# saidwivedi/TokenHMR

Hardware: AMD Instinct MI355X
Metric: crops_per_sec (higher is better)
Workload: dtype f32 (fp32 in / accumulate / out; the ViT GEMMs multiply each fp32 operand as three bf16 pieces on the bf16 MFMA pipe, six products per pair: `vit_gemm` split3; the fp32-MFMA mode is `exact_f32_mode`); 1 GPU; TokenHMR full path (ViT-H/16 + 6-layer token decoder + VQ lookup/decode + SMPL LBS), 256x256 crops, random-init weights; batch_per_gpu=64, global_batch=64, vit_depth=32, parallelism=dp1, allgather_outputs=False, vit_gemm=split3, ranks=1

## Files before the change

include/tokenhmr_hip.h:

```cpp
#ifndef TOKENHMR_HIP_H
#define TOKENHMR_HIP_H

#include <stddef.h>
#include <stdint.h>

#ifdef __cplusplus
extern "C" {
#endif

#define THMR_ABI_VERSION 5

typedef enum {
    THMR_OK = 0,
    THMR_ERR_INVALID = -1,
    THMR_ERR_HIP = -2,
    THMR_ERR_STATE = -3,
    THMR_ERR_NOMEM = -4,
    THMR_ERR_UNSUPPORTED = -5
} thmr_status;

typedef struct thmr_engine thmr_engine;

typedef struct {
    int32_t abi_version;
// ... 34 lines not shown
} thmr_smpl_desc;

typedef struct {
    float*   pred_cam;
    float*   rotmat;
    float*   betas;
    float*   cls_logits_softmax;
    float*   pred_cam_t;
    float*   focal_length;
    float*   pred_keypoints_3d;
    float*   pred_vertices;
    float*   pred_keypoints_2d;
    int32_t* token_idx;
    float*   vit_features;
    float*   token_out;
    float*   cls_logits;
    float*   pose6d;
} thmr_outputs;

enum {
    THMR_PROF_GEMM_QKV = 0, THMR_PROF_GEMM_PROJ = 1, THMR_PROF_GEMM_FC1 = 2, THMR_PROF_GEMM_FC2 = 3,
    THMR_PROF_ATTN = 4, THMR_PROF_LN = 5, THMR_PROF_PATCH = 6, THMR_PROF_DEC_KV = 7,
    THMR_PROF_HEAD = 8, THMR_PROF_LBS = 9, THMR_PROF_NUM = 10
};
typedef struct {
    double  ms;
    double  flops;
    double  bytes;
    int64_t launches;
} thmr_prof_entry;

int         thmr_abi_version(void);
const char* thmr_build_info(void);

int thmr_arena_bytes(const thmr_config* cfg, size_t* weight_bytes, size_t* scratch_bytes);

int thmr_mode_bytes(const thmr_config* cfg, int32_t vit_gemm_mode, size_t* split_weight_bytes, size_t* split_act_bytes, size_t* workspace_bytes);

int thmr_spec(const thmr_config* cfg, int32_t index, const char** name, int64_t* numel);

int thmr_create(const thmr_config* cfg, void* weight_arena_dev, void* scratch_arena_dev, thmr_engine** out);
void thmr_destroy(thmr_engine* e);
const char* thmr_last_error(const thmr_engine* e);

int thmr_load_weights(thmr_engine* e, const thmr_tensor_desc* tensors, size_t n, void* stream);
int thmr_load_smpl(thmr_engine* e, const thmr_smpl_desc* smpl, void* stream);
int thmr_finalize_weights(thmr_engine* e, int32_t assume_all_loaded, void* stream);
int thmr_weight_arena(thmr_engine* e, void** ptr_dev, size_t* bytes);

int thmr_forward(thmr_engine* e, const float* img_dev, int32_t B, const thmr_outputs* out, void* stream);

int thmr_engine_status(thmr_engine* e, void* stream);

int thmr_debug_decoder_timeline(thmr_engine* e, uint64_t* stamps_host, int32_t max_stamps, void* stream);

typedef enum {
    THMR_GEMM_F32_TILE = 0,
    THMR_GEMM_F32_TILE_SPLITK,
    THMR_GEMM_F32_RING,
    THMR_GEMM_F32_RING16,
    THMR_GEMM_S3_TILE,
    THMR_GEMM_S3_TILE_SPLITK,
    THMR_GEMM_S3_STREAM_WIDE,
    THMR_GEMM_S3_STREAM_NARROW,
    THMR_GEMM_S3_SPLITK_STREAM,
    THMR_GEMM_S3_RING
} thmr_gemm_kind;
enum { THMR_VIT_PATH_F32 = 0, THMR_VIT_PATH_SPLIT3 = 1, THMR_VIT_PATH_SPLIT3_SMALL = 2  };
enum { THMR_ATTN_F32 = 0, THMR_ATTN_F32_KEYSPLIT = 1, THMR_ATTN_F32_SPLIT3_OUT = 2, THMR_ATTN_B16 = 3 };
typedef struct thmr_gemm_choice {
    int32_t kind;
    int32_t ksplit;
} thmr_gemm_choice;
typedef struct thmr_vit_plan_desc {
    int32_t path;
    thmr_gemm_choice patch, qkv, proj, fc1, fc2, to_kv;
    int32_t attn;
    int32_t bs_blk;
    int32_t part2_in_scratch;
    int32_t tile_opts;
} thmr_vit_plan_desc;
int thmr_debug_vit_plan(const thmr_config* cfg, int32_t vit_gemm_mode, int32_t B, int32_t streams_available, thmr_vit_plan_desc* out);

int thmr_vit_forward(thmr_engine* e, const float* img_dev, int32_t B, float* feats_dev , void* stream);
int thmr_head_forward(thmr_engine* e, const float* ctx_dev , int32_t B, const thmr_outputs* out, void* stream);
int thmr_lbs_forward(thmr_engine* e, const float* rotmat_dev , const float* betas_dev ,
                     const float* cam_dev , int32_t B, float* verts_dev, float* joints_dev,
                     float* cam_t_dev, float* kp2d_dev, void* stream);
int thmr_vq_argmin(thmr_engine* e, const float* x_dev, int32_t rows, int32_t* idx_dev, float* dist_dev, void* stream);

int thmr_encode_tokens(thmr_engine* e, const float* pose_dev, int32_t B, int32_t* idx_dev, float* latent_dev, void* stream);
int thmr_vq_decode(thmr_engine* e, const float* probs_dev, int32_t B, float* pose6d_dev, void* stream);
int thmr_vq_decode_idx(thmr_engine* e, const int32_t* idx_dev, int32_t B, float* pose6d_dev, void* stream);
typedef struct thmr_tokenizer_out {
    int32_t* idx;
    float* latent;
    float* pose6d;
    float* rotmat;
    float* aa;
    float* commit_loss;
    float* perplexity;
    int32_t* code_count;
    int32_t accumulate_counts;
    int32_t reserved;
} thmr_tokenizer_out;
int thmr_tokenizer_roundtrip(thmr_engine* e, const float* pose6d_dev , int32_t B, const thmr_tokenizer_out* out, void* stream);

int thmr_op_gemm(const float* A_dev, int64_t lda, const float* W_dev, const float* bias_dev, const float* resid_dev,
                 float* C_dev, int64_t ldc, int32_t M, int32_t N, int32_t K, int32_t epi, float qscale, int32_t qcols,
                 int32_t variant, void* stream);
int thmr_op_split3(const float* src_dev, int64_t ld_src, void* dst_dev, int64_t ld_dst, int64_t rows, int32_t K, void* stream);
int thmr_op_gemm_split3(const void* A_split_dev, int64_t lda, const void* W_split_dev, int64_t ldw, const float* bias_dev,
                        const float* resid_dev, float* C_dev, int64_t ldc, int32_t M, int32_t N, int32_t K, int32_t epi,
                        float qscale, int32_t qcols, int32_t variant, void* stream);
int thmr_op_gemm_split3_out_split3(const void* A_split_dev, int64_t lda, const void* W_split_dev, int64_t ldw, const float* bias_dev,
                                   void* C_split_dev, int64_t ldcs, int32_t M, int32_t N, int32_t K, int32_t epi, float qscale,
                                   int32_t qcols, int32_t variant, void* stream);
int thmr_op_layernorm(const float* x_dev, const float* gamma_dev, const float* beta_dev, float* y_dev,
                      int32_t rows, int32_t D, float eps, int32_t relu, void* stream);
int thmr_op_vit_attention(const float* qkv_dev, float* out_dev , int32_t B, void* stream);
int thmr_op_vit_attention_variant(const float* qkv_dev, float* out_dev, int32_t B, int32_t variant, void* stream);
int thmr_op_vit_attention_split3(const float* qkv_dev, void* out_split_dev, int32_t B, void* stream);
int thmr_op_vit_attention_b16(const float* qkv_dev, void* out_dev, int32_t B, int32_t out_split, int32_t qt, void* stream);
int thmr_op_rot6d(const float* x_dev, float* R_dev, int32_t n, void* stream);
int thmr_op_aa_to_rotmat(const float* aa_dev, float* R_dev, int32_t n, void* stream);

int thmr_op_splitk_resid_ln(const float* part_dev, int32_t S, int32_t rows, int32_t D, const float* bias_dev, const float* resid_dev,
                            float* xout_dev, const float* gamma_dev, const float* beta_dev, void* y_dev, float eps, int32_t y_is_split3,
                            void* stream);
int thmr_op_add_ln64(const float* x_dev, const float* y_dev, const float* gamma_dev, const float* beta_dev, float* s_out_dev,
                     float* z_out_dev, int32_t rows, float eps, void* stream);
int thmr_op_transpose(const float* in_dev, float* out_dev, int32_t Bn, int32_t R, int32_t C, void* stream);
int thmr_op_softmax_argmax(const float* logits_dev, float* probs_or_null, int32_t* idx_or_null, int32_t rows, void* stream);
int thmr_op_cross_attn(const float* q_dev, const float* kv_dev, int64_t ldkv, int32_t koff, float* out_dev, int32_t B, void* stream);
int thmr_op_im2col_patch(const float* img_dev, void* A_dev, int32_t B, int32_t out_split, void* stream);
int thmr_op_conv3_gather(const float* in_dev, float* out_dev, const int32_t* src_or_null, int32_t Bn, int32_t Tin, int32_t Tout,
                         int32_t C, int32_t dil, int32_t prerelu, void* stream);
int thmr_op_conv_gather(const float* in_dev, float* out_dev, const int32_t* src_or_null, int32_t Bn, int32_t Tin, int32_t Tsrc,
                        int32_t Tout, int32_t C, int32_t Cp, int32_t ks, int32_t stride, int32_t pad, void* stream);
int thmr_op_conv_repack(const float* w_dev, float* wp_dev, int32_t co, int32_t ci, int32_t cp, int32_t kk, void* stream);
int thmr_op_vq_argmin_rows(const float* x_dev, const float* dot_dev, const float* cnorm_dev, int32_t* idx_dev, float* dist_or_null,
                           int32_t rows, void* stream);
int thmr_op_code_norm(const float* cb_dev, float* cn_dev, int32_t ncode, void* stream);
int thmr_op_vq_stats(const float* x_dev, const float* codebook_dev, const int32_t* idx_dev, int32_t rows, int32_t* code_count_dev,
                     int32_t accumulate, float* partial_scratch_dev, float* commit_or_null, float* perplexity_or_null, void* stream);
int thmr_op_rotmat_to_aa(const float* R_dev, float* aa_dev, int32_t n, void* stream);
int thmr_op_head_finish(int32_t kind, const float* ro_dev, int32_t ldro, const float* bpose_or_null, const float* init_pose_dev,
                        const float* init_betas_dev, const float* init_cam_dev, float* pose6d_or_null, float* rotmat_dev,
                        float* betas_dev, float* cam_dev, float* cam_t_or_null, float* focal_or_null, float focal_length, float img_size,
                        int32_t B, void* stream);
int thmr_op_decoder_init(const float* bias_dev, const float* pos_dev, float* x_dev, int32_t B, int32_t E, void* stream);

typedef struct thmr_smpl thmr_smpl;
int  thmr_smpl_create(const thmr_smpl_desc* desc, int32_t max_batch, int32_t device, thmr_smpl** out);
void thmr_smpl_destroy(thmr_smpl* m);
int  thmr_smpl_forward(thmr_smpl* m, const float* pose_dev, int32_t pose2rot, const float* betas_dev, int32_t B,
                       float* verts_dev , float* joints_dev , void* stream);

typedef struct thmr_smplh_desc {
    const float* v_template;
    const float* shapedirs;
    const float* posedirs;
    const float* J_regressor;
    const float* lbs_weights;
    const int32_t* parents;
    const int32_t* extra_verts;
    int32_t on_device;
    int32_t reserved;
} thmr_smplh_desc;
typedef struct thmr_smplh thmr_smplh;
int  thmr_smplh_create(const thmr_smplh_desc* desc, int32_t max_batch, int32_t device, thmr_smplh** out);
void thmr_smplh_destroy(thmr_smplh* m);
int  thmr_smplh_forward(thmr_smplh* m, const float* pose_dev, int32_t pose2rot, const float* betas_dev, const float* transl_dev,
                        int32_t body_only, int32_t B, float* verts_dev , float* joints_dev ,
                        void* stream);
#define THMR_MEAN_ROW_DIST_WS 256
int thmr_op_mean_row_dist(const float* a_dev, const float* b_dev, int32_t n_rows_per_item, int32_t row_lo, int32_t row_hi, int32_t B,
                          float* out_dev, float* workspace_dev, void* stream);

#define THMR_VAL_LOSS_PLAIN 0
#define THMR_VAL_LOSS_LOOSE 1
#define THMR_VAL_LOSS_WS_PER_ITEM 5
typedef struct thmr_val_loss_desc {
    double w_keypoints_2d, w_keypoints_3d, w_global_orient, w_body_pose, w_betas;
    double loose_weight;
    int32_t pelvis_id;
    int32_t mode;
    int32_t gt_pose_is_rotmat;
    int32_t reserved;
} thmr_val_loss_desc;
typedef struct thmr_val_loss_in {
    const float* pred_keypoints_2d;
    const float* pred_keypoints_3d;
    const float* pred_rotmat;
    const float* pred_betas;
    const float* gt_keypoints_2d;
    const float* gt_keypoints_3d;
    const float* gt_pose;
    const float* gt_betas;
    const float* has_global_orient;
    const float* has_body_pose;
    const float* has_betas;
    const float* valid_3d;
    const float* kp2d_thresh;
    const float* angle_thresh;
} thmr_val_loss_in;
typedef struct thmr_val_loss_out {
    float* losses;
    float* per_item;
    float* kp2d_err;
    float* angle_err;
    float* valid2d;
    float* weak2d;
    float* valid_rot;
    float* weak_rot;
    float* conf2d_used;
    float* conf3d_used;
// ... 142 lines not shown
```

tokenhmr_amd/_cabi.py:

```python
import ctypes as C
import os
import re

_HERE = os.path.dirname(os.path.abspath(__file__))
LIB_PATH = os.path.join(_HERE, "lib", "libtokenhmr_hip.so")
LIB_PATH_EXP = os.path.join(_HERE, "lib", "libtokenhmr_hip_exp.so")
HEADER = os.path.join(os.path.dirname(_HERE), "include", "tokenhmr_hip.h")

ABI_VERSION = 5
CFG_VIT_GEMM_F32, CFG_NO_PERSISTENT, CFG_HEAD_HMR2 = 1, 2, 8
PROF_NAMES = ["gemm_qkv", "gemm_proj", "gemm_fc1", "gemm_fc2", "attention", "layernorm", "patch_embed",
              "dec_kv", "head", "lbs"]


class Config(C.Structure):
    _fields_ = [("abi_version", C.c_int32), ("vit_depth", C.c_int32), ("dec_depth", C.c_int32),
                ("max_batch", C.c_int32), ("device", C.c_int32), ("flags", C.c_int32), ("reserved", C.c_int32 * 2)]


class TensorDesc(C.Structure):
    _fields_ = [("name", C.c_char_p), ("data", C.c_void_p), ("numel", C.c_int64),
                ("on_device", C.c_int32), ("reserved", C.c_int32)]


# ... 56 lines not shown


class JpegPlan(C.Structure):
    _fields_ = [(n, C.c_int32) for n in ("height", "width", "components", "h_samp", "v_samp", "win_x0", "win_y0", "win_w", "win_h", "mcu_row0",
                                         "mcu_rows_kept", "mcu_rows_decoded")] + \
               [(n, C.c_int32 * 3) for n in ("bx0", "by0", "bw", "bh", "coef_block")] + [("n_blocks", C.c_int32), ("quant", (C.c_uint16 * 64) * 3)]


class JpegItem(C.Structure):
    _fields_ = [("coef", C.c_void_p), ("plan", C.POINTER(JpegPlan)), ("win_x0", C.c_int32), ("win_y0", C.c_int32), ("win_w", C.c_int32),
                ("win_h", C.c_int32), ("out_dev", C.c_void_p), ("row_stride", C.c_int64)]


ERR_INVALID, ERR_HIP, ERR_STATE, ERR_NOMEM, ERR_UNSUPPORTED = -1, -2, -3, -4, -5

RENDER_MAX_LIGHTS = 16
RENDER_PER_IMAGE, RENDER_ONE_IMAGE = 0, 1
LIGHT_DIRECTIONAL, LIGHT_POINT = 0, 1


class RenderLight(C.Structure):
    _fields_ = [("type", C.c_int32), ("vec", C.c_float * 3), ("color", C.c_float * 3), ("intensity", C.c_float)]


class RenderDesc(C.Structure):
    _fields_ = [("width", C.c_int32), ("height", C.c_int32), ("fx", C.c_float), ("fy", C.c_float), ("cx", C.c_float), ("cy", C.c_float),
                ("znear", C.c_float), ("samples", C.c_int32), ("mode", C.c_int32), ("translate_first", C.c_int32),
                ("rot", C.c_float * 9), ("base_color", C.c_float * 3), ("mesh_colors", C.POINTER(C.c_float)), ("bg_color", C.c_float * 3),
                ("metallic", C.c_float), ("roughness", C.c_float), ("ambient", C.c_float * 3), ("n_lights", C.c_int32),
                ("lights", RenderLight * RENDER_MAX_LIGHTS), ("out_channels", C.c_int32), ("img_mean", C.c_float * 3),
                ("img_std", C.c_float * 3), ("ids_dev", C.c_void_p)]


SHEET_IMAGE, SHEET_FRONT, SHEET_SIDE = 1, 2, 4
SHEET_KEYPOINTS, SHEET_RECORDS, SHEET_RECORD_WORDS = 44, 49, 12


class SheetDesc(C.Structure):
    _fields_ = [("n", C.c_int32), ("width", C.c_int32), ("height", C.c_int32), ("img_res", C.c_int32), ("panels", C.c_int32),
                ("nrow", C.c_int32), ("padding", C.c_int32), ("canvas_width", C.c_int32), ("canvas_height", C.c_int32)]


class GemmChoice(C.Structure):
    _fields_ = [("kind", C.c_int32), ("ksplit", C.c_int32)]


GEMM_KINDS = ["f32_tile", "f32_tile_splitk", "f32_ring", "f32_ring16", "s3_tile", "s3_tile_splitk", "s3_stream_wide", "s3_stream_narrow",
              "s3_splitk_stream", "s3_ring"]
VIT_PATHS = ["f32", "split3", "split3_small"]
ATTN_KINDS = ["f32", "f32_keysplit", "f32_split3_out", "b16"]


class VitPlanDesc(C.Structure):
    _fields_ = [("path", C.c_int32)] + [(n, GemmChoice) for n in ("patch", "qkv", "proj", "fc1", "fc2", "to_kv")] + \
               [("attn", C.c_int32), ("bs_blk", C.c_int32), ("part2_in_scratch", C.c_int32), ("tile_opts", C.c_int32)]


class TokenizerOut(C.Structure):
    _fields_ = [("idx", C.c_void_p), ("latent", C.c_void_p), ("pose6d", C.c_void_p), ("rotmat", C.c_void_p), ("aa", C.c_void_p),
                ("commit_loss", C.c_void_p), ("perplexity", C.c_void_p), ("code_count", C.c_void_p), ("accumulate_counts", C.c_int32),
                ("reserved", C.c_int32)]


class ProfEntry(C.Structure):
    _fields_ = [("ms", C.c_double), ("flops", C.c_double), ("bytes", C.c_double), ("launches", C.c_int64)]


def declared_functions():
    with open(HEADER) as f:
        text = f.read()
    text = re.sub(r"/\*.*?\*/", "", text, flags=re.S)
    return {name: ret.strip() for ret, name in re.findall(r"([A-Za-z_][\w \t*]*?)\b(thmr_[a-z0-9_]+)\s*\(", text)}


def declared_symbols():
    return sorted(declared_functions())


_libs = {}

ROWOPS_SYMBOLS = ("thmr_op_splitk_resid_ln", "thmr_op_add_ln64", "thmr_op_transpose", "thmr_op_softmax_argmax", "thmr_op_cross_attn",
                  "thmr_op_im2col_patch", "thmr_op_conv3_gather", "thmr_op_conv_gather", "thmr_op_conv_repack", "thmr_op_vq_argmin_rows",
                  "thmr_op_code_norm", "thmr_op_head_finish", "thmr_op_decoder_init")

TOKENIZER_RT_SYMBOLS = ("thmr_vq_decode_idx", "thmr_tokenizer_roundtrip", "thmr_op_vq_stats", "thmr_op_rotmat_to_aa")

SMPLH_SYMBOLS = ("thmr_smplh_create", "thmr_smplh_destroy", "thmr_smplh_forward", "thmr_op_mean_row_dist")

LOSS_SYMBOLS = ("thmr_val_loss", "thmr_op_token_ce")

FRAMES_SYMBOLS = ("thmr_cropper_run_frames",)

JPEG_SYMBOLS = ("thmr_jpeg_probe", "thmr_jpeg_entropy_decode", "thmr_jpeg_decode_host", "thmr_jpeg_create", "thmr_jpeg_destroy",
                "thmr_jpeg_last_error", "thmr_jpeg_decode_batch")


def load(exp=None):
    if exp is None:
        exp = os.environ.get("THMR_LIB", "") == "exp"
    if isinstance(exp, str):
        path = os.path.abspath(exp)
        exp = path
    else:
        exp = bool(exp)
        path = LIB_PATH_EXP if exp else LIB_PATH
    if exp in _libs:
        return _libs[exp]
    if not os.path.exists(path):
        raise RuntimeError(
            f"{path} not found: the HIP extension is not built. Run `python __graft_entry__.py` "
            "(hipcc --offload-arch=gfx950). There is no CPU fallback for the product path.")
    try:
        import torch
    except ImportError:
        pass
    lib = C.CDLL(path)
    declared = declared_functions()
    restypes = {"int": C.c_int, "void": None, "const char*": C.c_char_p}
    for name, ret in declared.items():
        if ret not in restypes:
            raise RuntimeError(f"tokenhmr_hip.h declares {name} as returning '{ret}': _cabi.load() knows {sorted(restypes)}")
        if hasattr(lib, name):
            getattr(lib, name).restype = restypes[ret]
    older = isinstance(exp, str) and lib.thmr_abi_version() in (3, 4)
    missing = [s for s in sorted(declared) if not hasattr(lib, s) and not (older and s in ("thmr_mode_bytes",))
               and not (isinstance(exp, str) and s in ("thmr_renderer_sheet", "thmr_debug_vit_plan") + ROWOPS_SYMBOLS + TOKENIZER_RT_SYMBOLS + FRAMES_SYMBOLS + JPEG_SYMBOLS)]
    if missing:
        raise RuntimeError(f"libtokenhmr_hip.so lacks symbols declared in tokenhmr_hip.h: {missing}")
    vp, i32, i64, f32, sz = C.c_void_p, C.c_int32, C.c_int64, C.c_float, C.c_size_t
    lib.thmr_last_error.argtypes = [vp]
    lib.thmr_arena_bytes.argtypes = [C.POINTER(Config), C.POINTER(sz), C.POINTER(sz)]
    lib.thmr_spec.argtypes = [C.POINTER(Config), i32, C.POINTER(C.c_char_p), C.POINTER(i64)]
    if hasattr(lib, "thmr_mode_bytes"):
        lib.thmr_mode_bytes.argtypes = [C.POINTER(Config), i32, C.POINTER(sz), C.POINTER(sz), C.POINTER(sz)]
    lib.thmr_create.argtypes = [C.POINTER(Config), vp, vp, C.POINTER(vp)]
    lib.thmr_destroy.argtypes = [vp]
    lib.thmr_load_weights.argtypes = [vp, C.POINTER(TensorDesc), sz, vp]
    lib.thmr_load_smpl.argtypes = [vp, C.POINTER(SmplDesc), vp]
    lib.thmr_finalize_weights.argtypes = [vp, i32, vp]
    lib.thmr_weight_arena.argtypes = [vp, C.POINTER(vp), C.POINTER(sz)]
    lib.thmr_forward.argtypes = [vp, vp, i32, C.POINTER(Outputs), vp]
    lib.thmr_engine_status.argtypes = [vp, vp]
    lib.thmr_debug_decoder_timeline.argtypes = [vp, C.POINTER(C.c_uint64), i32, vp]
    if hasattr(lib, "thmr_debug_vit_plan"):
        lib.thmr_debug_vit_plan.argtypes = [C.POINTER(Config), i32, i32, i32, C.POINTER(VitPlanDesc)]
    lib.thmr_vit_forward.argtypes = [vp, vp, i32, vp, vp]
    lib.thmr_head_forward.argtypes = [vp, vp, i32, C.POINTER(Outputs), vp]
    lib.thmr_lbs_forward.argtypes = [vp, vp, vp, vp, i32, vp, vp, vp, vp, vp]
    lib.thmr_vq_argmin.argtypes = [vp, vp, i32, vp, vp, vp]
    lib.thmr_encode_tokens.argtypes = [vp, vp, i32, vp, vp, vp]
    lib.thmr_vq_decode.argtypes = [vp, vp, i32, vp, vp]
    lib.thmr_op_gemm.argtypes = [vp, i64, vp, vp, vp, vp, i64, i32, i32, i32, i32, f32, i32, i32, vp]
    lib.thmr_op_layernorm.argtypes = [vp, vp, vp, vp, i32, i32, f32, i32, vp]
    lib.thmr_op_vit_attention.argtypes = [vp, vp, i32, vp]
    lib.thmr_op_vit_attention_variant.argtypes = [vp, vp, i32, i32, vp]
    lib.thmr_op_vit_attention_split3.argtypes = [vp, vp, i32, vp]
    lib.thmr_op_vit_attention_b16.argtypes = [vp, vp, i32, i32, i32, vp]
    lib.thmr_op_split3.argtypes = [vp, i64, vp, i64, i64, i32, vp]
    lib.thmr_op_gemm_split3.argtypes = [vp, i64, vp, i64, vp, vp, vp, i64, i32, i32, i32, i32, f32, i32, i32, vp]
    lib.thmr_op_gemm_split3_out_split3.argtypes = [vp, i64, vp, i64, vp, vp, i64, i32, i32, i32, i32, f32, i32, i32, vp]
    lib.thmr_op_rot6d.argtypes = [vp, vp, i32, vp]
    lib.thmr_op_aa_to_rotmat.argtypes = [vp, vp, i32, vp]
    if hasattr(lib, "thmr_op_splitk_resid_ln"):
        lib.thmr_op_splitk_resid_ln.argtypes = [vp, i32, i32, i32, vp, vp, vp, vp, vp, vp, f32, i32, vp]
        lib.thmr_op_add_ln64.argtypes = [vp, vp, vp, vp, vp, vp, i32, f32, vp]
        lib.thmr_op_transpose.argtypes = [vp, vp, i32, i32, i32, vp]
        lib.thmr_op_softmax_argmax.argtypes = [vp, vp, vp, i32, vp]
        lib.thmr_op_cross_attn.argtypes = [vp, vp, i64, i32, vp, i32, vp]
        lib.thmr_op_im2col_patch.argtypes = [vp, vp, i32, i32, vp]
        lib.thmr_op_conv3_gather.argtypes = [vp, vp, vp, i32, i32, i32, i32, i32, i32, vp]
        lib.thmr_op_conv_gather.argtypes = [vp, vp, vp, i32, i32, i32, i32, i32, i32, i32, i32, i32, vp]
        lib.thmr_op_conv_repack.argtypes = [vp, vp, i32, i32, i32, i32, vp]
        lib.thmr_op_vq_argmin_rows.argtypes = [vp, vp, vp, vp, vp, i32, vp]
        lib.thmr_op_code_norm.argtypes = [vp, vp, i32, vp]
        lib.thmr_op_head_finish.argtypes = [i32, vp, i32, vp, vp, vp, vp, vp, vp, vp, vp, vp, vp, f32, f32, i32, vp]
        lib.thmr_op_decoder_init.argtypes = [vp, vp, vp, i32, i32, vp]
    if hasattr(lib, "thmr_tokenizer_roundtrip"):
        lib.thmr_vq_decode_idx.argtypes = [vp, vp, i32, vp, vp]
        lib.thmr_tokenizer_roundtrip.argtypes = [vp, vp, i32, C.POINTER(TokenizerOut), vp]
        lib.thmr_op_vq_stats.argtypes = [vp, vp, vp, i32, vp, i32, vp, vp, vp, vp]
        lib.thmr_op_rotmat_to_aa.argtypes = [vp, vp, i32, vp]
    if hasattr(lib, "thmr_smplh_create"):
        lib.thmr_smplh_create.argtypes = [C.POINTER(SmplhDesc), i32, i32, C.POINTER(vp)]
        lib.thmr_smplh_destroy.argtypes = [vp]
        lib.thmr_smplh_forward.argtypes = [vp, vp, i32, vp, vp, i32, i32, vp, vp, vp]
        lib.thmr_op_mean_row_dist.argtypes = [vp, vp, i32, i32, i32, i32, vp, vp, vp]
    if hasattr(lib, "thmr_val_loss"):
        lib.thmr_val_loss.argtypes = [C.POINTER(ValLossDesc), C.POINTER(ValLossIn), i32, C.POINTER(ValLossOut), vp, vp]
        lib.thmr_op_token_ce.argtypes = [vp, vp, i32, vp, vp, vp]
    lib.thmr_smpl_create.argtypes = [C.POINTER(SmplDesc), i32, i32, C.POINTER(vp)]
    lib.thmr_smpl_destroy.argtypes = [vp]
    lib.thmr_smpl_forward.argtypes = [vp, vp, i32, vp, i32, vp, vp, vp]
    lib.thmr_eval_pose.argtypes = [vp, vp, i32, i32, vp, i32, i32, i32, vp, vp, i32, i32, vp, vp, vp, vp, vp]
    lib.thmr_regress_joints.argtypes = [vp, vp, i32, i32, i32, vp, vp]
    lib.thmr_cropper_create.argtypes = [i32, C.POINTER(vp)]
    lib.thmr_cropper_destroy.argtypes = [vp]
    lib.thmr_cropper_last_error.argtypes = [vp]
    lib.thmr_cropper_run.argtypes = [vp, vp, i32, i32, i64, C.POINTER(CropDesc), i32, i32, i32, C.POINTER(f32), C.POINTER(f32), vp, vp]
    if hasattr(lib, "thmr_cropper_run_frames"):
        lib.thmr_cropper_run_frames.argtypes = [vp, C.POINTER(FrameCrop), i32, i32, i32, C.POINTER(f32), C.POINTER(f32), vp, vp]
    if hasattr(lib, "thmr_jpeg_probe"):
        lib.thmr_jpeg_probe.argtypes = [vp, sz, C.POINTER(JpegInfo)]
        lib.thmr_jpeg_entropy_decode.argtypes = [vp, sz, C.POINTER(i32), vp, i64, C.POINTER(JpegPlan)]
        lib.thmr_jpeg_decode_host.argtypes = [vp, sz, C.POINTER(i32), i32, vp, i64]
        lib.thmr_jpeg_create.argtypes = [i32, C.POINTER(vp)]
        lib.thmr_jpeg_destroy.argtypes = [vp]
        lib.thmr_jpeg_last_error.argtypes = [vp]
        lib.thmr_jpeg_decode_batch.argtypes = [vp, C.POINTER(JpegItem), i32, i32, vp]
    lib.thmr_renderer_create.argtypes = [i32, vp, i32, i32, C.POINTER(vp)]
    lib.thmr_renderer_destroy.argtypes = [vp]
    lib.thmr_renderer_last_error.argtypes = [vp]
    lib.thmr_renderer_run.argtypes = [vp, C.POINTER(RenderDesc), vp, vp, i32, vp, vp, vp]
    if hasattr(lib, "thmr_renderer_sheet"):
        lib.thmr_renderer_sheet.argtypes = [vp, C.POINTER(SheetDesc), vp, vp, vp, vp, vp, vp, vp, vp]
    lib.thmr_pack_records.argtypes = [C.POINTER(Outputs), i32, vp, vp]
    lib.thmr_bcast_weights.argtypes = [vp, vp, i32, vp]
    lib.thmr_allgather_records.argtypes = [vp, vp, i32, vp, vp]
    lib.thmr_prof_enable.argtypes = [vp, i32]
    lib.thmr_set_vit_gemm.argtypes = [vp, i32, vp]
    lib.thmr_get_vit_gemm.argtypes = [vp]
    lib.thmr_prof_collect.argtypes = [vp, C.POINTER(ProfEntry), i32]
    if lib.thmr_abi_version() != ABI_VERSION and not older:
        raise RuntimeError("libtokenhmr_hip.so ABI version mismatch")
    _libs[exp] = lib
    return lib


class EngineError(RuntimeError):
    pass


def check(rc, engine=None, lib=None):
    if rc != 0:
        lib = lib if lib is not None else load()
        msg = lib.thmr_last_error(engine)
        raise EngineError(f"tokenhmr_hip error {rc}: {msg.decode() if msg else '?'}")


def raise_error(rc, what, msg, error=EngineError, by_code=None):
    raise (by_code or {}).get(rc, error)(f"{what} error {rc}: {msg.decode() if msg else '?'}")


class Handle:
    error, error_by_code, no_gpu_error = EngineError, None, RuntimeError

    @classmethod
    def cuda_device(cls, device, needs_gpu, resolve):
        import torch
        dev = torch.device(device)
        if dev.type != "cuda":
            raise cls.no_gpu_error(needs_gpu)
        return torch.device("cuda", torch.cuda.current_device()) if resolve and dev.index is None else dev

    def __init__(self, device, stem, needs_gpu, last_error=None):
        self.device = self.cuda_device(device, needs_gpu, resolve=False)
        self._needs_gpu = needs_gpu
        self.lib = load()
        self._stem, self._per_handle = stem, last_error is None
        self._last_error = getattr(self.lib, last_error or stem + "_last_error")
# ... 26 lines not shown
```

tokenhmr_amd/csrc/common.h:

```cpp
#pragma once
#include <hip/hip_runtime.h>
#include <stdint.h>

typedef float f32x4 __attribute__((ext_vector_type(4)));
typedef float f32x16 __attribute__((ext_vector_type(16)));

#include <cstdlib>
#ifdef THMR_EXPERIMENTS
inline const char* thmr_knob(const char* name) { return getenv(name); }
#else
inline const char* thmr_knob(const char*) { return nullptr; }
#endif

#define THMR_WAVE 64

enum GemmEpi {
    EPI_NONE = 0,
    EPI_BIAS = 1,
    EPI_BIAS_GELU = 2,
    EPI_BIAS_RELU = 3,
    EPI_BIAS_RESID = 4,
    EPI_BIAS_QSCALE = 5,
    EPI_BIAS_POS = 6,
    EPI_NUM = 7
// ... 149 lines not shown
    const uint32_t u2 = __float_as_uint(r2);
    L = (u2 + 0x7fffu + ((u2 >> 16) & 1u)) & 0xffff0000u;
    if (nan) H = M = L = 0x7fc00000u;
}
__device__ __forceinline__ void split3_of(float x, uint32_t& h, uint32_t& m, uint32_t& l) {
    uint32_t H, M, L;
    split3_hi(x, H, M, L);
    h = H >> 16; m = M >> 16; l = L >> 16;
}
__device__ __forceinline__ uint32_t cvt_pk_bf16(float lo, float hi) {
    typedef __bf16 bf16x2_t __attribute__((ext_vector_type(2)));
    typedef float f32x2_t __attribute__((ext_vector_type(2)));
    return __builtin_bit_cast(uint32_t, __builtin_convertvector(f32x2_t{lo, hi}, bf16x2_t));
}
__device__ __forceinline__ void split3_pair(float x0, float x1, uint32_t& H, uint32_t& M, uint32_t& L) {
#pragma clang fp contract(off)
    typedef float f32x2_t __attribute__((ext_vector_type(2)));
    H = cvt_pk_bf16(x0, x1);
    f32x2_t r = f32x2_t{x0, x1} - f32x2_t{__uint_as_float(H << 16), __uint_as_float(H & 0xffff0000u)};
    M = cvt_pk_bf16(r.x, r.y);
    r = r - f32x2_t{__uint_as_float(M << 16), __uint_as_float(M & 0xffff0000u)};
    L = cvt_pk_bf16(r.x, r.y);
}
__device__ __forceinline__ void store_split3_quad(char* row, int c, f32x4 v) {
    typedef uint32_t u32x2 __attribute__((ext_vector_type(2)));
    uint32_t H[2], M[2], L[2];
    split3_pair(v[0], v[1], H[0], M[0], L[0]);
    split3_pair(v[2], v[3], H[1], M[1], L[1]);
    char* o = row + (c >> 3) * 48 + (c & 4) * 2;
    *reinterpret_cast<u32x2*>(o) = u32x2{H[0], H[1]};
    *reinterpret_cast<u32x2*>(o + 16) = u32x2{M[0], M[1]};
    *reinterpret_cast<u32x2*>(o + 32) = u32x2{L[0], L[1]};
}

__device__ __forceinline__ void store_split3_oct(char* row, int c, f32x4 lo, f32x4 hi) {
    typedef uint32_t u32x4_t __attribute__((ext_vector_type(4)));
    uint32_t H[4], M[4], L[4];
    split3_pair(lo[0], lo[1], H[0], M[0], L[0]);
    split3_pair(lo[2], lo[3], H[1], M[1], L[1]);
    split3_pair(hi[0], hi[1], H[2], M[2], L[2]);
    split3_pair(hi[2], hi[3], H[3], M[3], L[3]);
    u32x4_t* o = reinterpret_cast<u32x4_t*>(row + (c >> 3) * 48);
    o[0] = u32x4_t{H[0], H[1], H[2], H[3]};
    o[1] = u32x4_t{M[0], M[1], M[2], M[3]};
    o[2] = u32x4_t{L[0], L[1], L[2], L[3]};
}

__device__ __forceinline__ float wave_sum(float v) {
#pragma unroll
    for (int o = 32; o > 0; o >>= 1) v += __shfl_xor(v, o, 64);
    return v;
}
__device__ __forceinline__ float wave_max(float v) {
#pragma unroll
    for (int o = 32; o > 0; o >>= 1) v = fmaxf(v, __shfl_xor(v, o, 64));
    return v;
}

__device__ __forceinline__ void st_dev(float* p, float v) { __hip_atomic_store(p, v, __ATOMIC_RELAXED, __HIP_MEMORY_SCOPE_AGENT); }
__device__ __forceinline__ float ld_dev(const float* p) { return __hip_atomic_load(p, __ATOMIC_RELAXED, __HIP_MEMORY_SCOPE_AGENT); }
__device__ __forceinline__ f32x4 ld_dev4(const float* p) {
    typedef float f32x2_t __attribute__((ext_vector_type(2)));
    union { unsigned long long u; f32x2_t f; } a, b;
    a.u = __hip_atomic_load(reinterpret_cast<const unsigned long long*>(p), __ATOMIC_RELAXED, __HIP_MEMORY_SCOPE_AGENT);
    b.u = __hip_atomic_load(reinterpret_cast<const unsigned long long*>(p) + 1, __ATOMIC_RELAXED, __HIP_MEMORY_SCOPE_AGENT);
    return f32x4{a.f.x, a.f.y, b.f.x, b.f.y};
}

struct MixerLayerW {
    const float *ln1w, *ln1b, *wt1, *bt1, *wt2, *bt2, *ln2w, *ln2b, *wc1, *bc1, *wc2, *bc2;
};
struct MixerParams {
    MixerLayerW L[4];
    const float *tln_w, *tln_b;
    const float *wn, *bn, *nln_w, *nln_b;
    const float* mt;
    float* out;
};


struct DecLayerW {
    const float *n0w, *n0b, *wv, *wo1, *bo1;
    const float *n1w, *n1b, *wq, *wo2, *bo2;
    const float *n2w, *n2b, *w1, *b1, *w2, *b2;
};
struct DecParams {
    DecLayerW L[6];
    const float *tok_bias, *pos;
    const float* kv;
    const float *ro_w, *ro_b, *mt_w, *mt_b;
    float *dx, *dv, *dq, *dca, *dff, *ro, *mt;
    unsigned* sync;
    unsigned* host_err;
    int64_t ldkv;
    int depth, B;
    int timeline;
    int debug_fail;
    int barrier_a2a;
    int max_blocks;
    MixerParams mx;
    float* mixy[2];
    int mixer_cluster;
};

constexpr int THMR_HEAD_TOKEN = 0, THMR_HEAD_HMR2 = 1;
constexpr int THMR_HMR2_RO_ROWS = 157, THMR_HMR2_RO_LD = 160;
int launch_decoder_fused(const DecParams& p, hipStream_t s, int head = THMR_HEAD_TOKEN);
int decoder_max_coresident_blocks(int device, int head = THMR_HEAD_TOKEN);
int launch_hmr2_finish(const float* ro, int ldro, const float* init_pose, const float* init_betas, const float* init_cam, float* pose6d,
                       float* rotmat, float* betas, float* cam, float* cam_t, float* focal, float focal_length, float img_size, int B,
                       hipStream_t s);

int launch_mixer_fused(const MixerParams& p, int B, hipStream_t s);

int launch_gemm(const GemmArgs& a, int epi, int variant, hipStream_t s);
int launch_gemm_splitk(const GemmArgs& a, int variant, int ksplit, float* part, hipStream_t s);
int launch_gemm_ring(const GemmArgs& a, int epi, int ring, int ksplit, float* part, hipStream_t s);
int launch_gemm_ring16(const GemmArgs& a, int epi, hipStream_t s);
int launch_split3(const float* src, int64_t ld_src, void* dst, int64_t ld_dst, int64_t rows, int K, hipStream_t s);
int launch_gemm_split3(const GemmArgs& a, int epi, int variant, hipStream_t s);
int launch_gemm_split3_splitk(const GemmArgs& a, int ksplit, float* part, hipStream_t s);
size_t gemm_split3_persist_ws_bytes();
bool gemm_split3_persist_ok(const GemmArgs& a);
int launch_gemm_split3_persist(const GemmArgs& a, int epi, int mode, void* ws, hipStream_t s);
bool gemm_split3_persist_narrow_ok(const GemmArgs& a);
int launch_gemm_split3_persist_narrow(const GemmArgs& a, int epi, void* ws, hipStream_t s);
int launch_gemm_split3_splitk_stream(const GemmArgs& a, int ksplit, float* part, void* ws, hipStream_t s);
int gemm_split3_persist_error(void* ws, hipStream_t s, unsigned* err_out);
int gemm_split3_persist_bind_host_err(void* ws, unsigned* const* host_err_slot, hipStream_t s);
void* gemm_split3_persist_op_ws(hipStream_t s);
int launch_split16_tiles(const GemmArgs& a, int epi, int shape, hipStream_t s);
int launch_split16_persist(const GemmArgs& a, int epi, void* ws, bool narrow, hipStream_t s);
int launch_split16_tiles_tail(const GemmArgs& a, int epi, int cus, bool tail8, hipStream_t s);
int launch_gemm_split3_ring(const GemmArgs& a, int epi, int ksplit, float* part, hipStream_t s);
int launch_layernorm_split3(const float* x, const float* g, const float* b, void* y_split, int rows, int D, float eps, hipStream_t s);
int launch_gemm_skinny(const GemmArgs& a, int epi, hipStream_t s);
int launch_vit_attention(const float* qkv, float* out, int B, hipStream_t s);
int launch_vit_attention_split3(const float* qkv, void* out_split, int B, hipStream_t s);
int launch_vit_attention_keysplit(const float* qkv, float* out, int B, hipStream_t s);
int launch_vit_attention_variant(const float* qkv, float* out, int B, int variant, hipStream_t s);
int launch_vit_attention_b16(const float* qkv, void* out, int B, bool out_split, int qt, hipStream_t s);
int launch_layernorm(const float* x, const float* g, const float* b, float* y, int rows, int D, float eps, int relu,
                     hipStream_t s);
int launch_splitk_epilogue(const GemmArgs& a, int epi, const float* part, int S, hipStream_t s);
int launch_splitk_resid_ln(const float* part, int S, int rows, int D, const float* bias, const float* resid, float* xout,
                           const float* gamma, const float* beta, float* y, float eps, hipStream_t s, bool y_is_split3 = false);
int launch_add_ln64(const float* x, const float* y, const float* g, const float* b, float* s_out, float* z_out, int rows,
                    float eps, hipStream_t s);
int launch_im2col_patch(const float* img, float* A, int B, hipStream_t s);
int launch_im2col_patch_split3(const float* img, void* A_split, int B, hipStream_t s);
int launch_transpose(const float* in, float* out, int Bn, int R, int C, hipStream_t s);
int launch_softmax_argmax2048(const float* logits, float* probs, int32_t* idx, int rows, hipStream_t s);
int launch_conv3_gather(const float* in, float* out, const int32_t* src, int Bn, int Tin, int Tout, int C, int dil,
                        int prerelu, hipStream_t s);
int launch_conv_repack(const float* w, float* wp, int co, int ci, int kk, hipStream_t s);
int launch_conv_gather_general(const float* in, float* out, const int32_t* src, int Bn, int Tin, int Tsrc, int Tout, int C,
                               int Cp, int ks, int stride, int pad, hipStream_t s);
int launch_conv_repack_pad(const float* w, float* wp, int co, int ci, int cp, int kk, hipStream_t s);
int launch_decoder_init(const float* bias, const float* pos, float* x, int B, int E, hipStream_t s);
int launch_cross_attn(const float* q, const float* kv, int64_t ldkv, int koff, float* out, int B, hipStream_t s);
int launch_assemble(const float* ro, int ldro, const float* bpose, const float* init_pose, const float* init_betas,
                    const float* init_cam, float* pose6d, float* rotmat, float* betas, float* cam, float* cam_t,
                    float* focal, float focal_length, float img_size, int B, hipStream_t s);
int launch_rot6d(const float* x, float* R, int n, hipStream_t s);
int launch_aa_to_rotmat(const float* aa, float* R, int n, hipStream_t s);
int launch_cam_t(const float* cam, float* cam_t, float focal_length, float img_size, int B, hipStream_t s);
int launch_vq_argmin_rows(const float* x, const float* dot, const float* cnorm, int32_t* idx, float* dist, int rows,
                          hipStream_t s);
int launch_code_norm(const float* cb, float* cn, int ncode, hipStream_t s);
int launch_vq_lookup(const int32_t* idx, const float* x, const float* cb, float* out, int B, unsigned* bad_flag, hipStream_t s);
int vq_stats_partials(int rows);
int launch_vq_stats(const float* x, const float* cb, const int32_t* idx, int rows, int32_t* count, int accumulate, float* partial,
                    float* commit, float* perplexity, unsigned* bad_flag, hipStream_t s);
int launch_rotmat_to_aa(const float* R, float* aa, int n, hipStream_t s);
int launch_eval_pose(const float* pred, const float* gt, int nj, int gt_stride, const int32_t* kp, int nkp, int pelvis_ind,
                     int pelvis_mode, float* mpjpe, float* re, float* pelv, int B, hipStream_t s);
int launch_eval_pve(const float* pv, const float* gv, const float* pelv, int nv, float* pve, int B, hipStream_t s);
int launch_regress_joints(const float* J, const float* verts, int nj, int nv, float* out, int B, hipStream_t s);
constexpr int kMeanRowDistWs = 256;
int launch_mean_row_dist(const float* a, const float* b, int n, int row_lo, int row_hi, int B, float* out, float* partial, hipStream_t s);
struct ValLossArgs {
    const float *pred_kp2d, *pred_kp3d, *pred_rotmat, *pred_betas;
    const float *gt_kp2d, *gt_kp3d, *gt_pose, *gt_betas;
    const float *has_global_orient, *has_body_pose, *has_betas;
    const float *valid_3d, *kp2d_thresh, *angle_thresh;
    float *losses, *per_item, *kp2d_err, *angle_err;
    float *valid2d, *weak2d, *valid_rot, *weak_rot;
    float *conf2d_used, *conf3d_used, *has_betas_used;
    double* running;
    float* partial;
    double w[5];
// ... 36 lines not shown
```

tokenhmr_amd/csrc/decoder_fused.hip:

```cpp
#include <cstdlib>

#include "mixer_device.h"

namespace {

constexpr int E = 1024, INNER = 512, DMLP = 1024, TOKK = 192, NHEAD = 8;
constexpr int NBLK = 64, NWAVE = 8, NS = 8;
constexpr float LN_EPS = 1e-5f;

struct GridSync {
    unsigned* w;
    unsigned base;
    unsigned n;
    unsigned* host_err;
    int a2a;
};

template <class PF>
__device__ __forceinline__ bool grid_barrier(GridSync& gs, int tid, volatile int* s_ok, PF&& pf) {
    asm volatile("s_waitcnt vmcnt(0) lgkmcnt(0)" ::: "memory");
    pf();
    __syncthreads();
    gs.n += 1;
    const unsigned epoch = gs.base + gs.n;
// ... 164 lines not shown
                if (m < B) {
                    float o = v[r];
                    if constexpr (EPI != 0) o = o + bv;
                    if constexpr (EPI == 2) o = gelu_erf(o);
                    if constexpr (EPI == 4) o = ld_dev(resid + (int64_t)m * ldc + n) + o;
                    st_dev(C + (int64_t)m * ldc + n, o);
                }
            }
        }
        __syncthreads();
    }
}

__device__ __forceinline__ void gemv_multi(const float* __restrict__ A, const float* __restrict__ W0, const float* __restrict__ b0, float* C0,
                                           const float* __restrict__ W1, const float* __restrict__ b1, float* C1, int n_ro, int n_all, int B,
                                           float (*red)[64][4], int tid, bool dev_c1) {
    const int lane = tid & 63, wave = __builtin_amdgcn_readfirstlane(tid >> 6), l15 = lane & 15, g = lane >> 4;
    const int kbeg = wave * (E / NWAVE);
    const int nsub = (B + 15) >> 4, G = gridDim.x;
    auto wptr = [&](int vt) -> const float* {
        return vt < n_ro ? W0 + (int64_t)min(vt * 16 + l15, 31) * E + kbeg + g * 4
                         : W1 + (int64_t)((vt - n_ro) * 16 + l15) * E + kbeg + g * 4;
    };
    const int lanes_of_b = min(nsub, G);
    for (int mt = blockIdx.x % lanes_of_b; mt < nsub; mt += lanes_of_b) {
        const int first = blockIdx.x / lanes_of_b, step = G / lanes_of_b;
        if (first >= step) continue;
        const int m0 = mt * 16;
        const float* ap = A + (int64_t)min(m0 + l15, B - 1) * E + kbeg + g * 4;
        f32x4 xq[NS], wq[NS], wn[NS];
#pragma unroll
        for (int s = 0; s < NS; ++s) xq[s] = ld_dev4(ap + s * 16);
        int vt = first;
        if (vt < n_all) {
            const float* wp = wptr(vt);
#pragma unroll
            for (int s = 0; s < NS; ++s) wq[s] = *reinterpret_cast<const f32x4*>(wp + s * 16);
        }
#pragma unroll 1
        for (; vt < n_all; vt += step) {
            const int nxt = vt + step;
            if (nxt < n_all) {
                const float* wp = wptr(nxt);
#pragma unroll
                for (int s = 0; s < NS; ++s) wn[s] = *reinterpret_cast<const f32x4*>(wp + s * 16);
            }
            f32x4 acc = {0.f, 0.f, 0.f, 0.f};
#pragma unroll
            for (int s = 0; s < NS; ++s)
#pragma unroll
                for (int t = 0; t < 4; ++t) acc = __builtin_amdgcn_mfma_f32_16x16x4f32(xq[s][t], wq[s][t], acc, 0, 0, 0);
            *reinterpret_cast<f32x4*>(&red[wave][lane][0]) = acc;
            __syncthreads();
            if (wave == 0) {
                f32x4 v = *reinterpret_cast<const f32x4*>(&red[0][lane][0]);
#pragma unroll
                for (int w = 1; w < NWAVE; ++w) v += *reinterpret_cast<const f32x4*>(&red[w][lane][0]);
                const bool ro = vt < n_ro;
                const int n = (ro ? vt : vt - n_ro) * 16 + l15, N = ro ? 31 : 10240, ldc = ro ? 32 : 10240;
                if (n < N) {
                    const float bv = (ro ? b0 : b1)[n];
                    float* C = ro ? C0 : C1;
#pragma unroll
                    for (int r = 0; r < 4; ++r) {
                        const int m = m0 + g * 4 + r;
                        if (m < B) {
                            if (!ro && dev_c1) st_dev(&C[(int64_t)m * ldc + n], v[r] + bv);
                            else C[(int64_t)m * ldc + n] = v[r] + bv;
                        }
                    }
                }
            }
            __syncthreads();
#pragma unroll
            for (int s = 0; s < NS; ++s) wq[s] = wn[s];
        }
    }
}

}

namespace {

__device__ __forceinline__ void cross_attn_stage(const DecParams& p, int layer, int tid, float* pl ) {
    const int lane = tid & 63, l15 = lane & 15, g = lane >> 4;
    const int gwave = __builtin_amdgcn_readfirstlane(tid >> 6) * gridDim.x + blockIdx.x;
    for (int item = gwave; item < p.B * NHEAD; item += gridDim.x * NWAVE) {
        const int b = item >> 3, h = item & 7;
        const f32x4 qv = ld_dev4(p.dq + (int64_t)b * INNER + h * 64 + l15 * 4);
        const float* kb = p.kv + (int64_t)b * TOKK * p.ldkv + layer * 2 * INNER + h * 64 + l15 * 4;
        float s3[3] = {0.f, 0.f, 0.f};
        const int64_t cstride = (int64_t)48 * p.ldkv;
        const float* kp = kb + (int64_t)g * p.ldkv;
        auto load8 = [&](const float* src, f32x4 (&dst)[12]) {
#pragma unroll
            for (int i = 0; i < 12; ++i) dst[i] = *reinterpret_cast<const f32x4*>(src + (int64_t)(i * 4) * p.ldkv);
        };
        auto score8 = [&](const f32x4 (&kk)[12], int c) {
#pragma unroll
            for (int i = 0; i < 12; ++i) {
                float d = kk[i][0] * qv[0];
                d = fmaf(kk[i][1], qv[1], d);
                d = fmaf(kk[i][2], qv[2], d);
                d = fmaf(kk[i][3], qv[3], d);
                d += __shfl_xor(d, 1, 64);
                d += __shfl_xor(d, 2, 64);
                d += __shfl_xor(d, 4, 64);
                d += __shfl_xor(d, 8, 64);
                const int idx = c * 12 + i;
                const bool mine = l15 == (idx & 15);
                const float sv = d * 0.125f;
                if (mine && (idx >> 4) == 0) s3[0] = sv;
                if (mine && (idx >> 4) == 1) s3[1] = sv;
                if (mine && (idx >> 4) == 2) s3[2] = sv;
            }
        };
        {
            f32x4 ka[12], kc[12];
            load8(kp, ka);
#pragma unroll 1
            for (int c = 0; c < 4; c += 2) {
                load8(kp + (int64_t)(c + 1) * cstride, kc);
                score8(ka, c);
                if (c + 2 < 4) load8(kp + (int64_t)(c + 2) * cstride, ka);
                score8(kc, c + 1);
            }
        }
        const float m = wave_max(fmaxf(fmaxf(s3[0], s3[1]), s3[2]));
        float e3[3];
#pragma unroll
        for (int j = 0; j < 3; ++j) {
            e3[j] = expf(s3[j] - m);
            pl[g * 48 + j * 16 + l15] = e3[j];
        }
        const float sum = wave_sum((e3[0] + e3[1]) + e3[2]);
        const float* vp = kb + INNER + (int64_t)g * p.ldkv;
        const float* wl = pl + g * 48;
        f32x4 acc = {0.f, 0.f, 0.f, 0.f};
        auto pv8 = [&](const f32x4 (&vv)[12], int c) {
#pragma unroll
            for (int i = 0; i < 12; ++i) {
                const float w = wl[c * 12 + i];
#pragma unroll
                for (int e = 0; e < 4; ++e) acc[e] = fmaf(w, vv[i][e], acc[e]);
            }
        };
        {
            f32x4 va[12], vc[12];
            load8(vp, va);
#pragma unroll 1
            for (int c = 0; c < 4; c += 2) {
                load8(vp + (int64_t)(c + 1) * cstride, vc);
                pv8(va, c);
                if (c + 2 < 4) load8(vp + (int64_t)(c + 2) * cstride, va);
                pv8(vc, c + 1);
            }
        }
#pragma unroll
        for (int e = 0; e < 4; ++e) {
            acc[e] += __shfl_xor(acc[e], 16, 64);
            acc[e] += __shfl_xor(acc[e], 32, 64);
        }
        if (g == 0) {
            const float inv = 1.0f / sum;
            float* o = p.dca + (int64_t)b * INNER + h * 64 + l15 * 4;
#pragma unroll
            for (int e = 0; e < 4; ++e) st_dev(o + e, acc[e] * inv);
        }
    }
}

__device__ __forceinline__ bool mixer_cluster_stage(const DecParams& p, GridSync& gs, int tid, volatile int* s_ok, float* Y, float* U, float* Xl,
                                                    float* redbuf) {
    using namespace mixer;
    const int lane = tid & 63, wave = __builtin_amdgcn_readfirstlane(tid >> 6), l15 = lane & 15, g = lane >> 4;
    const int wg = blockIdx.x;
    const int per_crop = p.mixer_cluster, tpw = 10 / per_crop;
    const bool active = wg < per_crop * p.B;
    const int b = wg / per_crop, t0 = (wg - b * per_crop) * tpw * 16, nrow = tpw * 16;
    if (active) {
        f32x4 o[5];
        trans_ln<true>(p.mt + (int64_t)b * (T * H), p.mx.tln_w, p.mx.tln_b, redbuf, tid, lane, wave, o);
#pragma unroll
        for (int i = 0; i < 5; ++i) {
            const int e0 = (i * NT + tid) * 4, t = e0 >> 6, h = e0 & 63;
            if (t >= t0 && t < t0 + nrow) *reinterpret_cast<f32x4*>(&Xl[(t - t0) * LD + h]) = o[i];
        }
    }
    __syncthreads();
#pragma unroll 1
    for (int l = 0; l < 4; ++l) {
        const MixerLayerW& w = p.mx.L[l];
        float* yg = p.mixy[l & 1] + (int64_t)b * (T * H);
        if (active) {
            const float gamma = w.ln1w[lane], beta = w.ln1b[lane];
            for (int r = wave; r < nrow; r += NW) st_dev(yg + (t0 + r) * H + lane, ln_row_value(Xl[r * LD + lane], gamma, beta));
        }
        if (!grid_barrier(gs, tid, s_ok)) return false;
        if (active) {
            for (int idx = tid; idx < T * H / 4; idx += NT) {
                const int t = idx >> 4, h = (idx & 15) * 4;
                *reinterpret_cast<f32x4*>(&Y[t * LD + h]) = ld_dev4(yg + idx * 4);
            }
            __syncthreads();
#pragma unroll 1
            for (int tile = wave; tile < 16; tile += NW) token_mix1_tile(Y, U, w, tile, l15, g);
            __syncthreads();
#pragma unroll 1
            for (int tile = wave; tile < 4 * tpw; tile += NW) {
                const int tt = tile >> 2;
                token_mix2_tile(U, Xl + tt * 16 * LD, Y + (t0 + tt * 16) * LD, w, (tile & 3) * 16, t0 + tt * 16, l15, g);
            }
            __syncthreads();
#pragma unroll 1
            for (int tt = 0; tt < tpw; ++tt)
                channel_mix_tile_8waves(Y + (t0 + tt * 16) * LD, Xl + tt * 16 * LD, U, w, wave, lane, l15, g);
        }
    }
    if (active)
        for (int tt = wave; tt < tpw; tt += NW) norm_layer_tile(Xl + tt * 16 * LD, p.mx.out + ((int64_t)b * T + t0 + tt * 16) * H, p.mx, l15, g);
    return true;
}

template <int HEAD>
__global__ __launch_bounds__(NWAVE * 64) void decoder_persistent_kernel(DecParams p) {
    constexpr bool TOKEN = HEAD == THMR_HEAD_TOKEN;
    __shared__ __attribute__((aligned(16))) float mixY[TOKEN ? mixer::T * mixer::LD : 4];
    __shared__ __attribute__((aligned(16))) float mixU[TOKEN ? mixer::H * mixer::LD : 4];
    __shared__ __attribute__((aligned(16))) float mixX[TOKEN ? 80 * mixer::LD : 4];
    __shared__ float mixred[mixer::NW];
    static_assert(mixer::NW == NWAVE, "the distributed mixer tail uses the decoder kernel's 8 waves");
    __shared__ __attribute__((aligned(16))) float red[NWAVE][64][4];
    __shared__ RowStat rowstat;
    __shared__ unsigned s_base;
    __shared__ int s_ok;
    const int tid = threadIdx.x;
    if (tid == 0) s_base = __hip_atomic_load(&p.sync[1], __ATOMIC_RELAXED, __HIP_MEMORY_SCOPE_AGENT);
    __syncthreads();
    GridSync gs{p.sync, s_base, 0, p.host_err, p.barrier_a2a};
    bool ok = true;
#ifdef THMR_EXPERIMENTS
    if (p.debug_fail && blockIdx.x == 0 && tid == 0) {
        __hip_atomic_store(&gs.w[3], 1u, __ATOMIC_RELAXED, __HIP_MEMORY_SCOPE_AGENT);
        if (gs.host_err) __hip_atomic_store(gs.host_err, 1u, __ATOMIC_RELAXED, __HIP_MEMORY_SCOPE_SYSTEM);
    }
#endif
    const int B = p.B;
    unsigned long long* stamp = (p.timeline && blockIdx.x == 0 && tid == 0) ? reinterpret_cast<unsigned long long*>(p.sync + 16) : nullptr;
    int nstamp = 0;
#define THMR_STAMP() do { if (stamp) stamp[nstamp++] = wall_clock64(); } while (0)
    THMR_STAMP();

    for (int i = blockIdx.x * (NWAVE * 64) + tid; i < B * E; i += gridDim.x * NWAVE * 64) {
        const int c = i & (E - 1);
        st_dev(p.dx + i, p.tok_bias[c] + p.pos[c]);
    }
    THMR_STAMP();
    WPre pre;
    pre.item = -1;
    ok = grid_barrier(gs, tid, &s_ok, [&] { prefetch_w(pre, p.L[0].wv, E, INNER, B, tid); });
    THMR_STAMP();
    for (int l = 0; ok && l < p.depth; ++l) {
        const DecLayerW& w = p.L[l];
        gemv_stage<true, 0>(p.dx, E, w.n0w, w.n0b, w.wv, E, nullptr, nullptr, p.dv, INNER, INNER, B, red, &rowstat, tid, pre);
        THMR_STAMP();
        if (!(ok = grid_barrier(gs, tid, &s_ok, [&] { prefetch_w(pre, w.wo1, INNER, E, B, tid); }))) break;
        THMR_STAMP();
        gemv_stage<false, 4>(p.dv, INNER, nullptr, nullptr, w.wo1, INNER, w.bo1, p.dx, p.dx, E, E, B, red, &rowstat, tid, pre);
        THMR_STAMP();
        if (!(ok = grid_barrier(gs, tid, &s_ok, [&] { prefetch_w(pre, w.wq, E, INNER, B, tid); }))) break;
        THMR_STAMP();
        gemv_stage<true, 0>(p.dx, E, w.n1w, w.n1b, w.wq, E, nullptr, nullptr, p.dq, INNER, INNER, B, red, &rowstat, tid, pre);
        THMR_STAMP();
        pre.item = -1;
        if (!(ok = grid_barrier(gs, tid, &s_ok))) break;
        THMR_STAMP();
        cross_attn_stage(p, l, tid, &red[__builtin_amdgcn_readfirstlane(tid >> 6)][0][0]);
        THMR_STAMP();
        if (!(ok = grid_barrier(gs, tid, &s_ok, [&] { prefetch_w(pre, w.wo2, INNER, E, B, tid); }))) break;
        THMR_STAMP();
        gemv_stage<false, 4>(p.dca, INNER, nullptr, nullptr, w.wo2, INNER, w.bo2, p.dx, p.dx, E, E, B, red, &rowstat, tid, pre);
        THMR_STAMP();
        if (!(ok = grid_barrier(gs, tid, &s_ok, [&] { prefetch_w(pre, w.w1, E, DMLP, B, tid); }))) break;
        THMR_STAMP();
        gemv_stage<true, 2>(p.dx, E, w.n2w, w.n2b, w.w1, E, w.b1, nullptr, p.dff, DMLP, DMLP, B, red, &rowstat, tid, pre);
        THMR_STAMP();
        if (!(ok = grid_barrier(gs, tid, &s_ok, [&] { prefetch_w(pre, w.w2, DMLP, E, B, tid); }))) break;
        THMR_STAMP();
        gemv_stage<false, 4>(p.dff, DMLP, nullptr, nullptr, w.w2, DMLP, w.b2, p.dx, p.dx, E, E, B, red, &rowstat, tid, pre);
        THMR_STAMP();
        if (l + 1 < p.depth) {
            if (!(ok = grid_barrier(gs, tid, &s_ok, [&] { prefetch_w(pre, p.L[l + 1].wv, E, INNER, B, tid); }))) break;
        } else {
            pre.item = -1;
            if (!(ok = grid_barrier(gs, tid, &s_ok))) break;
        }
        THMR_STAMP();
    }
    if constexpr (!TOKEN) {
        if (ok) gemv_stage<false, 1>(p.dx, E, nullptr, nullptr, p.ro_w, E, p.ro_b, nullptr, p.ro, THMR_HMR2_RO_LD, THMR_HMR2_RO_LD, B, red, &rowstat, tid, pre);
        THMR_STAMP();
    } else {
        if (ok) {
            gemv_multi(p.dx, p.ro_w, p.ro_b, p.ro, p.mt_w, p.mt_b, p.mt, 2, 2 + 640, B, red, tid, p.mixer_cluster != 0);
        }
        THMR_STAMP();
        if (ok && p.mixer_cluster != 0) {
            ok = grid_barrier(gs, tid, &s_ok);
            if (ok) ok = mixer_cluster_stage(p, gs, tid, &s_ok, mixY, mixU, mixX, mixred);
        }
        THMR_STAMP();
    }
    __syncthreads();
    if (tid == 0) {
        const unsigned old = __hip_atomic_fetch_add(&p.sync[2], 1u, __ATOMIC_ACQ_REL, __HIP_MEMORY_SCOPE_AGENT);
        if (old == gridDim.x - 1) {
            __hip_atomic_store(&p.sync[1], gs.base + gs.n, __ATOMIC_RELAXED, __HIP_MEMORY_SCOPE_AGENT);
            __hip_atomic_store(&p.sync[2], 0u, __ATOMIC_RELEASE, __HIP_MEMORY_SCOPE_AGENT);
        }
    }
}

}

constexpr int kDecMinGrid = 128;
int launch_decoder_fused(const DecParams& p, hipStream_t s, int head) {
    if (p.B < 1 || p.depth < 1 || p.depth > 6) return -1;
    if (head == THMR_HEAD_HMR2) {
        if (p.mixer_cluster != 0) return -1;
        const int nsub = (p.B + 15) / 16;
        int grid = NBLK * (nsub < 4 ? nsub : 4);
        if (p.max_blocks > 0 && grid > p.max_blocks) grid = p.max_blocks;
        if (grid > 256) grid = 256;
        hipLaunchKernelGGL(decoder_persistent_kernel<THMR_HEAD_HMR2>, dim3(grid), dim3(NWAVE * 64), 0, s, p);
        return hipGetLastError() == hipSuccess ? 0 : -2;
    }
    if (head != THMR_HEAD_TOKEN) return -1;
    const int nsub = (p.B + 15) / 16;
    int grid = NBLK * (nsub < 4 ? nsub : 4);
    static const int min_grid = [] { const char* e = thmr_knob("THMR_DEC_MIN_GRID"); return e ? atoi(e) : kDecMinGrid; }();
    if (grid < min_grid) grid = min_grid;
    if (p.mixer_cluster != 0 && p.mixer_cluster != 10 && p.mixer_cluster != 5 && p.mixer_cluster != 2) return -1;
    if (grid < p.mixer_cluster * p.B) grid = p.mixer_cluster * p.B;
    if (p.max_blocks > 0 && grid > p.max_blocks) grid = p.max_blocks;
    if (grid > 256) grid = 256;
    if (grid < p.mixer_cluster * p.B) return -1;
#ifdef THMR_EXPERIMENTS
    static const bool coop = [] { const char* e = thmr_knob("THMR_DEC_COOP"); return e && e[0] == '1'; }();
    if (coop) {
        DecParams pc = p;
        void* args[] = {&pc};
        return hipLaunchCooperativeKernel(reinterpret_cast<const void*>(&decoder_persistent_kernel<THMR_HEAD_TOKEN>), dim3(grid), dim3(NWAVE * 64), args, 0, s) == hipSuccess ? 0 : -2;
    }
#endif
    hipLaunchKernelGGL(decoder_persistent_kernel<THMR_HEAD_TOKEN>, dim3(grid), dim3(NWAVE * 64), 0, s, p);
    return hipGetLastError() == hipSuccess ? 0 : -2;
}

int decoder_max_coresident_blocks(int device, int head) {
    int cus = 0, per_cu = 0;
    if (hipDeviceGetAttribute(&cus, hipDeviceAttributeMultiprocessorCount, device) != hipSuccess || cus < 1) return -2;
    const hipError_t q = head == THMR_HEAD_HMR2
        ? hipOccupancyMaxActiveBlocksPerMultiprocessor(&per_cu, decoder_persistent_kernel<THMR_HEAD_HMR2>, NWAVE * 64, 0)
        : hipOccupancyMaxActiveBlocksPerMultiprocessor(&per_cu, decoder_persistent_kernel<THMR_HEAD_TOKEN>, NWAVE * 64, 0);
    if (q != hipSuccess || per_cu < 1) return -2;
    return cus;
}
```

tokenhmr_amd/csrc/engine.hip:

```cpp
#include <hip/hip_runtime.h>

#include <cmath>
#include <cstdio>
#include <cstdlib>
#include <cstring>
#include <map>
#include <mutex>
#include <string>
#include <unordered_map>
#include <vector>

#include "../../include/tokenhmr_hip.h"
#include "abi_util.h"
#include "common.h"
#include "vit_plan.h"

namespace {

constexpr int HEADS = 16;
constexpr int E = 1024, DEC_MLP = 1024;
constexpr int TN = 160, NCLS = 2048, HID = 64, HID_INTER = 256, TOK_INTER = 64, MIX = 4;
constexpr int CODE = 256, VQW = 512, VQJ = 21;
constexpr float VIT_EPS = 1e-6f, LN_EPS = 1e-5f;
constexpr int kFusedHeadMaxB = 128;
// ... 573 lines not shown
            if (plan.attn == THMR_ATTN_F32_KEYSPLIT) LAUNCH_OK(launch_vit_attention_keysplit(big, h, B, st));
            else LAUNCH_OK(launch_vit_attention(big, h, B, st));
        }
        if (int rc = resid_linear_ln(THMR_PROF_GEMM_PROJ, plan.proj, h, DIM, w.pw, w.pb, w.n2w, w.n2b, h)) return rc;
        {
            ProfScope ps(e, st, THMR_PROF_GEMM_FC1, 2.0 * M * DIM * (double)MLP, 4.0 * ((double)M * DIM + (double)DIM * MLP + (double)M * MLP), (i & 3) == 0);
            GemmArgs a = mk(h, DIM, w.f1w, DIM, w.f1b, nullptr, 0, big, MLP, M, MLP, DIM);
            LAUNCH_OK(run_gemm(e, plan.fc1, a, EPI_BIAS_GELU, nullptr, st));
        }
        if (int rc = resid_linear_ln(THMR_PROF_GEMM_FC2, plan.fc2, big, MLP, w.f2w, w.f2b, nxt_w, nxt_b, last && feats_out ? feats_out : h))
            return rc;
    }
    return 0;
}


int vq_tiny_variant(const thmr_engine* e, int B) { return (e->tiny_gemm && B * TOK <= kSmallM) ? 11 : -1; }

int vq_decode_convs(thmr_engine* e, int B, float* bpose, hipStream_t st) {
    auto& so = e->so;
    const int tv = vq_tiny_variant(e, B);
    float* G[2] = {e->S(so.gat), e->S(so.gat2)};
    float *x0 = e->S(so.act0), *x1 = e->S(so.act1), *hid = e->S(so.act2);
    const int32_t* inv = reinterpret_cast<const int32_t*>(e->warena + e->o_inv);
    auto scatter = [&](GemmArgs& a, float* dst, const int32_t* table, int tin, int tout, int dil, int relu) {
        a.cs_out = dst; a.cs_inv = table; a.cs_tin = tin; a.cs_tout = tout; a.cs_dil = dil; a.cs_relu = relu;
    };
    auto conv = [&](int id, const float* opnd, int T, const float* bias, float* plain) {
        const int ci = kConv3Ci[id], co = kConv3Co[id];
        return mk(opnd, 3 * ci, e->warena + e->convp[id], 3 * ci, bias, nullptr, 0, plain, co, B * T, co, 3 * ci);
    };
    int cur = 0;
    {
        GemmArgs a = conv(0, G[cur], 160, e->hot.conv_b[0], nullptr);
        scatter(a, G[cur ^ 1], inv + 0 * 160, 160, e->vq_len[1], 1, 0);
        LAUNCH_OK(launch_gemm(a, EPI_BIAS_RELU, tv, st));
        cur ^= 1;
    }
    for (int i = 0; i < 4; ++i) {
        const int T = e->vq_len[i + 1];
        GemmArgs a = conv(1 + i, G[cur], T, e->hot.conv_b[1 + i], i == 3 ? x0 : nullptr);
        if (i < 3) scatter(a, G[cur ^ 1], inv + (i + 1) * 160, T, e->vq_len[i + 2], 1, 0);
        else scatter(a, G[cur ^ 1], nullptr, VQJ, VQJ, 3, 1);
        LAUNCH_OK(launch_gemm(a, EPI_BIAS_RELU, tv, st));
        cur ^= 1;
    }
    const int Tq = VQJ;
    float* res = x0;
    float* nres = x1;
    for (int blk = 0; blk < 2; ++blk) {
        {
            GemmArgs a = conv(5 + blk, G[cur], Tq, e->hot.conv_b[5 + blk], hid);
            LAUNCH_OK(launch_gemm(a, EPI_BIAS_RELU, tv, st));
        }
        GemmArgs a = mk(hid, VQW, e->hot.res_w[blk], VQW, e->hot.res_b[blk], res, VQW, blk == 0 ? nres : nullptr, VQW, B * Tq, VQW, VQW);
        scatter(a, G[cur ^ 1], nullptr, Tq, Tq, 1, blk == 0 ? 1 : 0);
        LAUNCH_OK(launch_gemm(a, EPI_BIAS_RESID, tv, st));
        cur ^= 1;
        std::swap(res, nres);
    }
    {
        GemmArgs a = conv(7, G[cur], Tq, e->hot.conv_b[7], nullptr);
        scatter(a, G[cur ^ 1], nullptr, Tq, Tq, 1, 0);
        LAUNCH_OK(launch_gemm(a, EPI_BIAS, tv, st));
        cur ^= 1;
    }
    GemmArgs a = conv(8, G[cur], Tq, e->hot.conv_b[8], bpose);
    LAUNCH_OK(launch_gemm(a, EPI_BIAS, tv, st));
    return 0;
}

int vq_decode(thmr_engine* e, const float* probs, int B, float* bpose, hipStream_t st) {
    GemmArgs a = mk(probs, NCLS, e->warena + e->o_cbT, NCLS, nullptr, nullptr, 0, nullptr, CODE, B * TN, CODE, NCLS);
    a.cs_out = e->S(e->so.gat); a.cs_inv = nullptr; a.cs_tin = 160; a.cs_tout = 160; a.cs_dil = 1; a.cs_relu = 0;
    LAUNCH_OK(launch_gemm(a, EPI_NONE, vq_tiny_variant(e, B), st));
    return vq_decode_convs(e, B, bpose, st);
}

int vq_decode_idx(thmr_engine* e, const int32_t* idx, const float* x, int B, float* bpose, hipStream_t st) {
    LAUNCH_OK(launch_vq_lookup(idx, x, e->W("quantizer.codebook"), e->S(e->so.gat), B, e->host_err ? e->host_err + 2 : nullptr, st));
    return vq_decode_convs(e, B, bpose, st);
}

int head_forward(thmr_engine* e, const float* ctx, int B, const thmr_outputs* out, hipStream_t st) {
    auto& so = e->so;
    const int M = B * TOK;
    float* big = e->S(so.big);
    const int ldkv = e->dec_depth * 2 * INNER;
    {
        ProfScope ps(e, st, THMR_PROF_DEC_KV, 2.0 * M * DIM * (double)ldkv, 4.0 * ((double)M * DIM + (double)ldkv * DIM + (double)M * ldkv));
        const VitPlan plan = plan_of(e, B);
        if (plan.to_kv.kind != THMR_GEMM_F32_TILE) {
            LAUNCH_OK(launch_split3(ctx, DIM, e->split_act, DIM, M, DIM, st));
            GemmArgs a = mk(reinterpret_cast<const float*>(e->split_act), DIM, reinterpret_cast<const float*>(e->kv_s), DIM, nullptr, nullptr, 0, big, ldkv, M, ldkv, DIM);
            a.tile_opts = plan.tile_opts;
            LAUNCH_OK(run_gemm(e, plan.to_kv, a, EPI_NONE, nullptr, st));
        } else {
            GemmArgs a = mk(ctx, DIM, e->warena + e->o_kv_all, DIM, nullptr, nullptr, 0, big, ldkv, M, ldkv, DIM);
            LAUNCH_OK(run_gemm(e, plan.to_kv, a, EPI_NONE, nullptr, st));
        }
    }
    ProfScope ps_head(e, st, THMR_PROF_HEAD, e->hmr2 ? 2.0 * B * (6.0 * 4.2e6 + 0.16e6) : 2.0 * B * (6.0 * 4.2e6 + 116.7e6 + 167.8e6 + 705.0e6), 0);
    float *dx = e->S(so.dx), *dh = e->S(so.dh), *dv = e->S(so.dv), *dq = e->S(so.dq), *dca = e->S(so.dca), *dff = e->S(so.dff);
    const std::string T = "smpl_head.transformer.";
    const std::string C = "smpl_head.decpose.";
    float* ro = e->S(so.ro);
    float *mt = e->S(so.mt), *cf = e->S(so.cf), *cf2 = e->S(so.cf2);
    const bool fused_head = !e->legacy_head && B <= kFusedHeadMaxB;
    bool mixer_in_decoder = false;
    if (fused_head) {
        DecParams d = e->dec;
        d.B = B;
        if (e->hmr2) {
            d.mixer_cluster = 0;
            LAUNCH_OK(launch_decoder_fused(d, st, THMR_HEAD_HMR2));
        } else {
            const int slots = d.max_blocks < 256 ? d.max_blocks : 256;
            d.mixer_cluster = !e->mixer_cluster ? 0 : 10 * B <= slots ? 10 : 5 * B <= slots ? 5 : 2 * B <= slots ? 2 : 0;
            mixer_in_decoder = d.mixer_cluster != 0;
            d.mx = e->mix;
            d.mixy[0] = cf; d.mixy[1] = cf2;
            LAUNCH_OK(launch_decoder_fused(d, st));
        }
    } else {
    LAUNCH_OK(launch_decoder_init(e->W(T + "to_token_embedding.bias"), e->W(T + "pos_embedding"), dx, B, E, st));
    for (int l = 0; l < e->dec_depth; ++l) {
        const std::string p = T + "transformer.layers." + std::to_string(l) + ".";
        LAUNCH_OK(launch_layernorm(dx, e->W(p + "0.norm.weight"), e->W(p + "0.norm.bias"), dh, B, E, LN_EPS, 0, st));
        {
            GemmArgs a = mk(dh, E, e->W(p + "0.fn.to_qkv.weight") + (size_t)2 * INNER * E, E, nullptr, nullptr, 0, dv, INNER, B, INNER, E);
            LAUNCH_OK(launch_gemm_skinny(a, EPI_NONE, st));
        }
        {
            GemmArgs a = mk(dv, INNER, e->W(p + "0.fn.to_out.0.weight"), INNER, e->W(p + "0.fn.to_out.0.bias"), dx, E, dx, E, B, E, INNER);
            LAUNCH_OK(launch_gemm_skinny(a, EPI_BIAS_RESID, st));
        }
        LAUNCH_OK(launch_layernorm(dx, e->W(p + "1.norm.weight"), e->W(p + "1.norm.bias"), dh, B, E, LN_EPS, 0, st));
        {
            GemmArgs a = mk(dh, E, e->W(p + "1.fn.to_q.weight"), E, nullptr, nullptr, 0, dq, INNER, B, INNER, E);
            LAUNCH_OK(launch_gemm_skinny(a, EPI_NONE, st));
        }
        LAUNCH_OK(launch_cross_attn(dq, big, ldkv, l * 2 * INNER, dca, B, st));
        {
            GemmArgs a = mk(dca, INNER, e->W(p + "1.fn.to_out.0.weight"), INNER, e->W(p + "1.fn.to_out.0.bias"), dx, E, dx, E, B, E, INNER);
            LAUNCH_OK(launch_gemm_skinny(a, EPI_BIAS_RESID, st));
        }
        LAUNCH_OK(launch_layernorm(dx, e->W(p + "2.norm.weight"), e->W(p + "2.norm.bias"), dh, B, E, LN_EPS, 0, st));
        {
            GemmArgs a = mk(dh, E, e->W(p + "2.fn.net.0.weight"), E, e->W(p + "2.fn.net.0.bias"), nullptr, 0, dff, DEC_MLP, B, DEC_MLP, E);
            LAUNCH_OK(launch_gemm_skinny(a, EPI_BIAS_GELU, st));
        }
        {
            GemmArgs a = mk(dff, DEC_MLP, e->W(p + "2.fn.net.3.weight"), DEC_MLP, e->W(p + "2.fn.net.3.bias"), dx, E, dx, E, B, E, DEC_MLP);
            LAUNCH_OK(launch_gemm_skinny(a, EPI_BIAS_RESID, st));
        }
    }
    if (e->hmr2) {
        GemmArgs a = mk(dx, E, e->warena + e->o_ro_w, E, e->warena + e->o_ro_b, nullptr, 0, ro, THMR_HMR2_RO_LD, B, THMR_HMR2_RO_LD, E);
        LAUNCH_OK(launch_gemm_skinny(a, EPI_BIAS, st));
    } else {
        {
            GemmArgs a = mk(dx, E, e->warena + e->o_ro_w, E, e->warena + e->o_ro_b, nullptr, 0, ro, 32, B, 31, E);
            LAUNCH_OK(launch_gemm_skinny(a, EPI_BIAS, st));
        }
        {
            GemmArgs a = mk(dx, E, e->W(C + "mixer_trans.ff.0.weight"), E, e->W(C + "mixer_trans.ff.0.bias"), nullptr, 0, mt, TN * HID, B, TN * HID, E);
            LAUNCH_OK(launch_gemm_skinny(a, EPI_BIAS, st));
        }
    }
    }
    if (out && out->token_out) HIP_OK(hipMemcpyAsync(out->token_out, dx, sizeof(float) * B * E, hipMemcpyDeviceToDevice, st));
    if (e->hmr2) {
        float* rot = (out && out->rotmat) ? out->rotmat : e->S(so.rot);
        float* betas = (out && out->betas) ? out->betas : e->S(so.betas);
        float* cam = (out && out->pred_cam) ? out->pred_cam : e->S(so.cam);
        float* camt = (out && out->pred_cam_t) ? out->pred_cam_t : e->S(so.camt);
        LAUNCH_OK(launch_hmr2_finish(ro, THMR_HMR2_RO_LD, e->hot.init_pose, e->hot.init_betas, e->hot.init_cam, out ? out->pose6d : nullptr,
                                     rot, betas, cam, camt, out ? out->focal_length : nullptr, FOCAL, IMG, B, st));
        return 0;
    }
    const int R = B * TN;
    float *nl = e->S(so.nl), *nl2 = e->S(so.nl2);
    if (fused_head) {
        if (!mixer_in_decoder) LAUNCH_OK(launch_mixer_fused(e->mix, B, st));
    } else {
        LAUNCH_OK(launch_layernorm(mt, e->W(C + "mixer_trans.ff.1.weight"), e->W(C + "mixer_trans.ff.1.bias"), cf, B, TN * HID, LN_EPS, 1, st));
        for (int m = 0; m < MIX; ++m) {
            const std::string p = C + "mixer_head." + std::to_string(m) + ".";
            float *y1 = e->S(so.y1), *tT = e->S(so.tT), *u = e->S(so.u), *yt = e->S(so.yt), *y = e->S(so.y), *s = e->S(so.s),
                  *z0 = e->S(so.z0), *zh = e->S(so.zh);
            LAUNCH_OK(launch_layernorm(cf, e->W(p + "layernorm1.weight"), e->W(p + "layernorm1.bias"), y1, R, HID, LN_EPS, 0, st));
            LAUNCH_OK(launch_transpose(y1, tT, B, TN, HID, st));
            {
                GemmArgs a = mk(tT, TN, e->W(p + "MLP_token.ff.0.weight"), TN, e->W(p + "MLP_token.ff.0.bias"), nullptr, 0, u, TOK_INTER, B * HID, TOK_INTER, TN);
                LAUNCH_OK(launch_gemm(a, EPI_BIAS_GELU, -1, st));
// ... 439 lines not shown
    char* p = e->split_w;
    for (int i = 0; i < e->vit_depth; ++i) {
        const VitBlockW& w = e->vitw[i];
        auto conv = [&](const float* src, int rows, int K, const char*& out) -> int {
            out = p;
            const int rc = launch_split3(src, K, p, K, rows, K, st);
            p += (size_t)rows * K * 6;
            return rc;
        };
        LAUNCH_OK(conv(w.qkvw, 3 * DIM, DIM, e->vitw_s[i].qkv));
        LAUNCH_OK(conv(w.pw, DIM, DIM, e->vitw_s[i].proj));
        LAUNCH_OK(conv(w.f1w, MLP, DIM, e->vitw_s[i].fc1));
        LAUNCH_OK(conv(w.f2w, DIM, MLP, e->vitw_s[i].fc2));
    }
    e->kv_s = p;
    LAUNCH_OK(launch_split3(e->warena + e->o_kv_all, DIM, p, DIM, (int64_t)kv_rows, DIM, st));
    p += kv_rows * DIM * 6;
    e->pe_s = p;
    LAUNCH_OK(launch_split3(e->hot.pe_w, 768, p, 768, DIM, 768, st));
    return 0;
}

int thmr_finalize_weights(thmr_engine* e, int32_t assume_all_loaded, void* stream) {
    if (!e) return fail(e, THMR_ERR_INVALID, "null engine");
    hipStream_t st = static_cast<hipStream_t>(stream);
    if (!assume_all_loaded) {
        for (auto& n : e->required)
            if (!e->slots[n].loaded) return fail(e, THMR_ERR_STATE, "missing tensor '" + n + "' (strict load)");
        if (!e->smpl_loaded) return fail(e, THMR_ERR_STATE, "SMPL constants not loaded (thmr_load_smpl)");
    }
    int32_t* flags = reinterpret_cast<int32_t*>(e->warena + e->o_flags);
    if (!assume_all_loaded) {
        if (int r = write_arena_constants(e, st)) return r;
        size_t enc_loaded = 0;
        for (auto& n : e->enc_names) enc_loaded += e->slots[n].loaded ? 1 : 0;
        if (enc_loaded != 0 && enc_loaded != e->enc_names.size())
            return fail(e, THMR_ERR_STATE, "tokenizer encoder partially loaded: " + std::to_string(enc_loaded) + " of " +
                                               std::to_string(e->enc_names.size()) + " tensors");
        e->enc_ready = !e->hmr2 && enc_loaded == e->enc_names.size();
    } else {
        int32_t f[2] = {0, 0};
        HIP_OK(hipMemcpyAsync(f, flags, sizeof(f), hipMemcpyDeviceToHost, st));
        HIP_OK(hipStreamSynchronize(st));
        if (f[1] != (e->hmr2 ? kArenaMagicHmr2 : kArenaMagic))
            return fail(e, THMR_ERR_STATE, "thmr_finalize_weights(assume_all_loaded=1): the weight arena does not carry a loaded model "
                                           "(no loader magic word of this head kind): was it broadcast before the root called thmr_load_weights, or never received?");
        e->enc_ready = !e->hmr2 && f[0] == kEncMagic;
    }
    if (!e->hmr2) {
        for (int i = 0; i < 9; ++i)
            LAUNCH_OK(launch_conv_repack(e->W(std::string(kConv3[i]) + ".weight"), e->warena + e->convp[i], kConv3Co[i], kConv3Ci[i], 3, st));
        LAUNCH_OK(launch_transpose(e->W("quantizer.codebook"), e->warena + e->o_cbT, 1, NCLS, CODE, st));
        LAUNCH_OK(launch_code_norm(e->W("quantizer.codebook"), e->warena + e->o_cnorm, NCLS, st));
    }
    LAUNCH_OK(e->smpl.derive(e->warena, st));
    if (e->enc_ready)
        for (int i = 0; i < kEncN; ++i)
            if (kEnc[i].ks > 1)
                LAUNCH_OK(launch_conv_repack_pad(e->W(std::string(kEnc[i].name) + ".weight"), e->warena + e->enc_convp[i],
                                                 kEnc[i].co, kEnc[i].ci, kEnc[i].cp, kEnc[i].ks, st));
    e->vitw.resize(e->vit_depth);
    for (int i = 0; i < e->vit_depth; ++i) {
        const std::string p = "backbone.blocks." + std::to_string(i) + ".";
        VitBlockW& w = e->vitw[i];
        w.n1w = e->W(p + "norm1.weight"); w.n1b = e->W(p + "norm1.bias");
        w.qkvw = e->W(p + "attn.qkv.weight"); w.qkvb = e->W(p + "attn.qkv.bias");
        w.pw = e->W(p + "attn.proj.weight"); w.pb = e->W(p + "attn.proj.bias");
        w.n2w = e->W(p + "norm2.weight"); w.n2b = e->W(p + "norm2.bias");
        w.f1w = e->W(p + "mlp.fc1.weight"); w.f1b = e->W(p + "mlp.fc1.bias");
        w.f2w = e->W(p + "mlp.fc2.weight"); w.f2b = e->W(p + "mlp.fc2.bias");
    }
    {
        DecParams& d = e->dec;
        const std::string T = "smpl_head.transformer.";
        for (int l = 0; l < e->dec_depth; ++l) {
            const std::string p = T + "transformer.layers." + std::to_string(l) + ".";
            DecLayerW& w = d.L[l];
            w.n0w = e->W(p + "0.norm.weight"); w.n0b = e->W(p + "0.norm.bias");
            w.wv = e->W(p + "0.fn.to_qkv.weight") + (size_t)2 * INNER * E;
            w.wo1 = e->W(p + "0.fn.to_out.0.weight"); w.bo1 = e->W(p + "0.fn.to_out.0.bias");
            w.n1w = e->W(p + "1.norm.weight"); w.n1b = e->W(p + "1.norm.bias");
            w.wq = e->W(p + "1.fn.to_q.weight");
            w.wo2 = e->W(p + "1.fn.to_out.0.weight"); w.bo2 = e->W(p + "1.fn.to_out.0.bias");
            w.n2w = e->W(p + "2.norm.weight"); w.n2b = e->W(p + "2.norm.bias");
            w.w1 = e->W(p + "2.fn.net.0.weight"); w.b1 = e->W(p + "2.fn.net.0.bias");
            w.w2 = e->W(p + "2.fn.net.3.weight"); w.b2 = e->W(p + "2.fn.net.3.bias");
        }
        d.tok_bias = e->W(T + "to_token_embedding.bias"); d.pos = e->W(T + "pos_embedding");
        d.kv = e->S(e->so.big); d.ldkv = (int64_t)e->dec_depth * 2 * INNER;
        d.ro_w = e->warena + e->o_ro_w; d.ro_b = e->warena + e->o_ro_b;
        if (!e->hmr2) { d.mt_w = e->W("smpl_head.decpose.mixer_trans.ff.0.weight"); d.mt_b = e->W("smpl_head.decpose.mixer_trans.ff.0.bias"); }
        d.dx = e->S(e->so.dx); d.dv = e->S(e->so.dv); d.dq = e->S(e->so.dq); d.dca = e->S(e->so.dca); d.dff = e->S(e->so.dff);
        d.ro = e->S(e->so.ro); d.mt = e->S(e->so.mt);
        d.sync = reinterpret_cast<unsigned*>(e->S(e->so.sync));
        d.depth = e->dec_depth; d.B = 0;
        { const char* tl = thmr_knob("THMR_DEC_TIMELINE"); d.timeline = tl && tl[0] == '1'; }
        { const char* ft = thmr_knob("THMR_DEC_FORCE_TIMEOUT"); d.debug_fail = ft && ft[0] == '1'; }
        { const char* bm = thmr_knob("THMR_DEC_BARRIER"); d.barrier_a2a = bm && bm[0] == '1'; }
        {
            const int nb = decoder_max_coresident_blocks(e->cfg.device, e->hmr2 ? THMR_HEAD_HMR2 : THMR_HEAD_TOKEN);
            if (nb < 1) return fail(e, THMR_ERR_HIP, "persistent decoder kernel cannot be resident on this device (occupancy query failed)");
            d.max_blocks = nb;
            d.host_err = e->host_err;
        }
        MixerParams& m = e->mix;
        const std::string C = "smpl_head.decpose.";
        for (int i = 0; i < (e->hmr2 ? 0 : MIX); ++i) {
            const std::string p = C + "mixer_head." + std::to_string(i) + ".";
            MixerLayerW& w = m.L[i];
            w.ln1w = e->W(p + "layernorm1.weight"); w.ln1b = e->W(p + "layernorm1.bias");
            w.wt1 = e->W(p + "MLP_token.ff.0.weight"); w.bt1 = e->W(p + "MLP_token.ff.0.bias");
            w.wt2 = e->W(p + "MLP_token.ff.3.weight"); w.bt2 = e->W(p + "MLP_token.ff.3.bias");
            w.ln2w = e->W(p + "layernorm2.weight"); w.ln2b = e->W(p + "layernorm2.bias");
            w.wc1 = e->W(p + "MLP_channel.ff.0.weight"); w.bc1 = e->W(p + "MLP_channel.ff.0.bias");
            w.wc2 = e->W(p + "MLP_channel.ff.3.weight"); w.bc2 = e->W(p + "MLP_channel.ff.3.bias");
        }
        if (!e->hmr2) {
            m.tln_w = e->W(C + "mixer_trans.ff.1.weight"); m.tln_b = e->W(C + "mixer_trans.ff.1.bias");
            m.wn = e->W(C + "mixer_norm_layer.ff.0.weight"); m.bn = e->W(C + "mixer_norm_layer.ff.0.bias");
            m.nln_w = e->W(C + "mixer_norm_layer.ff.1.weight"); m.nln_b = e->W(C + "mixer_norm_layer.ff.1.bias");
            m.mt = e->S(e->so.mt); m.out = e->S(e->so.nl2);
        }
        auto& h = e->hot;
        h.pe_w = e->W("backbone.patch_embed.proj.weight"); h.pe_b = e->W("backbone.patch_embed.proj.bias");
        h.pos = e->W("backbone.pos_embed");
        h.lastn_w = e->W("backbone.last_norm.weight"); h.lastn_b = e->W("backbone.last_norm.bias");
        if (!e->hmr2) { h.cls_w = e->W(C + "class_pred_layer.weight"); h.cls_b = e->W(C + "class_pred_layer.bias"); }
        h.init_pose = e->W("smpl_head.init_body_pose"); h.init_betas = e->W("smpl_head.init_betas"); h.init_cam = e->W("smpl_head.init_cam");
        for (int i = 0; i < (e->hmr2 ? 0 : 9); ++i) h.conv_b[i] = e->W(std::string(kConv3[i]) + ".bias");
        for (int b = 0; b < (e->hmr2 ? 0 : 2); ++b) {
            const std::string p = "decoder.decoder.14.0.model." + std::to_string(b) + ".";
            h.res_w[b] = e->W(p + "conv2.weight"); h.res_b[b] = e->W(p + "conv2.bias");
        }
    }
    if (e->vit_gemm_mode == 1) {
        if (int r = build_split_weights(e, st)) return r;
        HIP_OK(hipStreamSynchronize(st));
    }
    e->finalized = true;
    return 0;
}

int thmr_set_vit_gemm(thmr_engine* e, int32_t mode, void* stream) {
    if (!e) return fail(e, THMR_ERR_INVALID, "null engine");
    if (mode != 0 && mode != 1) return fail(e, THMR_ERR_INVALID, "vit gemm mode must be 0 (exact-fp32 MFMA) or 1 (split3 on the bf16 matrix pipe)");
    if (mode == 1) {
        if (!e->finalized) return fail(e, THMR_ERR_STATE, "thmr_set_vit_gemm(1) needs finalized weights (thmr_finalize_weights)");
        if (hipSetDevice(e->cfg.device) != hipSuccess) return fail(e, THMR_ERR_HIP, "hipSetDevice failed");
        if (int r = build_split_weights(e, static_cast<hipStream_t>(stream))) return r;
        HIP_OK(hipStreamSynchronize(static_cast<hipStream_t>(stream)));
    }
    e->vit_gemm_mode = mode;
    return 0;
}

int thmr_get_vit_gemm(thmr_engine* e) { return e ? e->vit_gemm_mode : -1; }

static int refuse_hmr2(thmr_engine* e, const char* what) {
    return fail(e, THMR_ERR_INVALID, std::string(what) + " does not exist on an engine created with THMR_CFG_HEAD_HMR2 (the HMR2 head has no pose tokens and no tokenizer)");
}
static int refuse_hmr2_outputs(thmr_engine* e, const thmr_outputs* out) {
    if (!e->hmr2 || !out) return 0;
    if (out->cls_logits_softmax) return refuse_hmr2(e, "thmr_outputs.cls_logits_softmax");
    if (out->cls_logits) return refuse_hmr2(e, "thmr_outputs.cls_logits");
    if (out->token_idx) return refuse_hmr2(e, "thmr_outputs.token_idx");
    return 0;
}

int thmr_vq_decode(thmr_engine* e, const float* probs_dev, int32_t B, float* pose6d_dev, void* stream) {
    if (int r = check_ready(e, B)) return r;
    if (e->hmr2) return refuse_hmr2(e, "thmr_vq_decode");
    if (!probs_dev || !pose6d_dev) return fail(e, THMR_ERR_INVALID, "null buffer");
// ... 63 lines not shown

static int report_bad_code_index(thmr_engine* e) {
    if (!e->host_err || *static_cast<volatile unsigned*>(e->host_err + 2) == 0) return 0;
    e->host_err[2] = 0;
    return fail(e, THMR_ERR_INVALID, "a code index outside [0, 2048) was passed to thmr_vq_decode_idx / thmr_tokenizer_roundtrip in an earlier "
                                     "call (clamped on the device, nothing was read out of bounds); that call's outputs are invalid");
}

int thmr_vq_decode_idx(thmr_engine* e, const int32_t* idx_dev, int32_t B, float* pose6d_dev, void* stream) {
    if (int r = check_ready(e, B)) return r;
    if (e->hmr2) return refuse_hmr2(e, "thmr_vq_decode_idx");
    if (int r = report_bad_code_index(e)) return r;
    if (!idx_dev || !pose6d_dev) return fail(e, THMR_ERR_INVALID, "null buffer");
    return vq_decode_idx(e, idx_dev, nullptr, B, pose6d_dev, static_cast<hipStream_t>(stream));
}

int thmr_tokenizer_roundtrip(thmr_engine* e, const float* pose6d_dev, int32_t B, const thmr_tokenizer_out* out, void* stream) {
    if (int r = check_ready(e, B, static_cast<hipStream_t>(stream))) return r;
    if (e->hmr2) return refuse_hmr2(e, "thmr_tokenizer_roundtrip");
    if (!e->enc_ready) return fail(e, THMR_ERR_STATE, "tokenizer encoder weights ('encoder.encoder.*') were not loaded");
    if (int r = report_bad_code_index(e)) return r;
    if (!pose6d_dev || !out) return fail(e, THMR_ERR_INVALID, "null buffer");
    if (out->accumulate_counts && !out->code_count) return fail(e, THMR_ERR_INVALID, "accumulate_counts needs a code_count buffer");
    hipStream_t st = static_cast<hipStream_t>(stream);
    int32_t* idx = out->idx ? out->idx : reinterpret_cast<int32_t*>(e->S(e->so.tokidx));
    const float* lat = nullptr;
    if (int r = encode_tokens_call(e, pose6d_dev, B, idx, out->latent, &lat, st)) return r;
    unsigned* flag = e->host_err ? e->host_err + 2 : nullptr;
    const float* cb = e->W("quantizer.codebook");
    if (out->commit_loss || out->perplexity || out->code_count) {
        float* sc = enc_scratch_a2(e, B) + (size_t)B * 320 * VQW;
        int32_t* cnt = out->code_count ? out->code_count : reinterpret_cast<int32_t*>(sc);
        LAUNCH_OK(launch_vq_stats(lat, cb, idx, B * TN, cnt, out->code_count && out->accumulate_counts, sc + NCLS, out->commit_loss,
                                  out->perplexity, flag, st));
    }
    float* pose = out->pose6d ? out->pose6d : e->S(e->so.bpose);
    if (int r = vq_decode_idx(e, idx, lat, B, pose, st)) return r;
    if (out->rotmat || out->aa) {
        float* rot = out->rotmat ? out->rotmat : e->S(e->so.rot);
        LAUNCH_OK(launch_rot6d(pose, rot, B * VQJ, st));
        if (out->aa) LAUNCH_OK(launch_rotmat_to_aa(rot, out->aa, B * VQJ, st));
    }
    return 0;
}

int thmr_weight_arena(thmr_engine* e, void** ptr_dev, size_t* bytes) {
    if (!e) return fail(e, THMR_ERR_INVALID, "null engine");
    if (ptr_dev) *ptr_dev = e->warena;
    if (bytes) *bytes = e->wfloats * sizeof(float);
    return 0;
}

int thmr_engine_status(thmr_engine* e, void* stream) {
    if (!e) return fail(e, THMR_ERR_INVALID, "null engine");
    hipStream_t st = static_cast<hipStream_t>(stream);
    unsigned words[4] = {0, 0, 0, 0};
    HIP_OK(hipMemcpyAsync(words, e->sarena + e->so.sync, sizeof(words), hipMemcpyDeviceToHost, st));
    HIP_OK(hipStreamSynchronize(st));
    if (words[3] != 0 || (e->host_err && *static_cast<volatile unsigned*>(e->host_err) != 0)) return recover_decoder_timeout(e);
    if (int r = report_bad_code_index(e)) return r;
    if (e->s3_ws) {
        unsigned err = 0;
        if (gemm_split3_persist_error(e->s3_ws, st, &err) != 0) return fail(e, THMR_ERR_HIP, "reading the split3 hand-over error word failed");
        if (e->s3_host_err && *static_cast<volatile unsigned*>(e->s3_host_err) != 0) err = 1;
#ifdef THMR_EXPERIMENTS
        if (e->s3_persist && e->vit_gemm_mode == 1 && !e->s3_forced_once) {
            const char* f = thmr_knob("THMR_SPLIT3_FORCE_TIMEOUT");
            if (f && f[0] == '1') { err = 1; e->s3_forced_once = true; }
        }
#endif
        if (err != 0) return recover_split3_timeout(e);
    }
    return 0;
}

int thmr_debug_decoder_timeline(thmr_engine* e, uint64_t* stamps_host, int32_t max_stamps, void* stream) {
    if (!e || !stamps_host || max_stamps < 1 || max_stamps > 240) return fail(e, THMR_ERR_INVALID, "bad argument");
    hipStream_t st = static_cast<hipStream_t>(stream);
    HIP_OK(hipMemcpyAsync(stamps_host, e->sarena + e->so.sync + 16, sizeof(uint64_t) * max_stamps, hipMemcpyDeviceToHost, st));
    HIP_OK(hipStreamSynchronize(st));
    return 0;
}

int thmr_debug_vit_plan(const thmr_config* cfg, int32_t vit_gemm_mode, int32_t B, int32_t streams_available, thmr_vit_plan_desc* out) {
    if (int r = validate_cfg(cfg)) return r;
    if (vit_gemm_mode != 0 && vit_gemm_mode != 1) return fail(nullptr, THMR_ERR_INVALID, "vit gemm mode must be 0 or 1");
    if (!out || B < 1 || B > cfg->max_batch) return fail(nullptr, THMR_ERR_INVALID, "null out / batch outside [1, max_batch]");
    thmr_engine tmp;
    tmp.max_batch = cfg->max_batch;
    layout_scratch(&tmp);
    VitPlanIn in{};
    in.mode = vit_gemm_mode; in.B = B; in.dec_depth = cfg->dec_depth;
    in.split_ready = vit_gemm_mode == 1 && cfg->max_batch >= kSplit3LowMinB;
    in.streams = streams_available != 0 && !(cfg->flags & THMR_CFG_NO_PERSISTENT);
    in.part_floats = tmp.so.part_floats;
    *out = plan_vit(read_knobs(), in);
    return 0;
}

static int end_turn(thmr_engine* e, Turn& turn, int r) {
    const int t = turn.end();
    if (r) return r;
    return t ? fail(e, THMR_ERR_HIP, "hipEventRecord failed at the end of the call (per-device engine turnstile)") : 0;
}
#define THMR_TURN(turn, e, st)                                                                                         \
    Turn turn(e, st);                                                                                                  \
    if (turn.rc) return fail(e, THMR_ERR_HIP, "the per-device engine turnstile could not create / wait for its event")

int thmr_vit_forward(thmr_engine* e, const float* img_dev, int32_t B, float* feats_dev, void* stream) {
    if (int r = check_ready(e, B, static_cast<hipStream_t>(stream))) return r;
    if (!img_dev || !feats_dev) return fail(e, THMR_ERR_INVALID, "null buffer");
    THMR_TURN(turn, e, static_cast<hipStream_t>(stream));
    return end_turn(e, turn, vit_forward(e, img_dev, B, feats_dev, static_cast<hipStream_t>(stream)));
}

static int head_forward_call(thmr_engine* e, const float* ctx_dev, int32_t B, const thmr_outputs* out, hipStream_t st) {
    if (int r = head_forward(e, ctx_dev, B, out, st)) return r;
    if (out && (out->pred_vertices || out->pred_keypoints_3d || out->pred_keypoints_2d)) {
        const float* rot = out->rotmat ? out->rotmat : e->S(e->so.rot);
        const float* betas = out->betas ? out->betas : e->S(e->so.betas);
        const float* camt = out->pred_cam_t ? out->pred_cam_t : e->S(e->so.camt);
        return lbs(e, rot, betas, camt, B, out->pred_vertices, out->pred_keypoints_3d, out->pred_keypoints_2d, st);
    }
    return 0;
}

int thmr_head_forward(thmr_engine* e, const float* ctx_dev, int32_t B, const thmr_outputs* out, void* stream) {
    if (int r = check_ready(e, B, static_cast<hipStream_t>(stream))) return r;
    if (!ctx_dev) return fail(e, THMR_ERR_INVALID, "null buffer");
    if (int r = refuse_hmr2_outputs(e, out)) return r;
    hipStream_t st = static_cast<hipStream_t>(stream);
    THMR_TURN(turn, e, st);
    return end_turn(e, turn, head_forward_call(e, ctx_dev, B, out, st));
}

static int forward_call(thmr_engine* e, const float* img_dev, int32_t B, const thmr_outputs* out, hipStream_t st) {
    float* ctx = e->S(e->so.h);
    if (int r = vit_forward(e, img_dev, B, nullptr, st)) return r;
    if (out->vit_features)
        HIP_OK(hipMemcpyAsync(out->vit_features, ctx, sizeof(float) * (size_t)B * TOK * DIM, hipMemcpyDeviceToDevice, st));
    if (int r = head_forward(e, ctx, B, out, st)) return r;
    const float* rot = out->rotmat ? out->rotmat : e->S(e->so.rot);
    const float* betas = out->betas ? out->betas : e->S(e->so.betas);
    const float* camt = out->pred_cam_t ? out->pred_cam_t : e->S(e->so.camt);
#ifdef THMR_EXPERIMENTS
    if (e->s3_ws && e->s3_persist && e->vit_gemm_mode == 1 && !e->s3_forced_once && e->s3_host_err) {
        const char* f = thmr_knob("THMR_SPLIT3_FORCE_TIMEOUT");
        if (f && f[0] == '2') { *e->s3_host_err = 1; e->s3_forced_once = true; }
    }
#endif
    return lbs(e, rot, betas, camt, B, out->pred_vertices, out->pred_keypoints_3d, out->pred_keypoints_2d, st);
}

int thmr_forward(thmr_engine* e, const float* img_dev, int32_t B, const thmr_outputs* out, void* stream) {
    if (int r = check_ready(e, B, static_cast<hipStream_t>(stream))) return r;
    if (!img_dev || !out) return fail(e, THMR_ERR_INVALID, "null buffer");
    if (int r = refuse_hmr2_outputs(e, out)) return r;
    hipStream_t st = static_cast<hipStream_t>(stream);
    THMR_TURN(turn, e, st);
    return end_turn(e, turn, forward_call(e, img_dev, B, out, st));
}

int thmr_lbs_forward(thmr_engine* e, const float* rotmat_dev, const float* betas_dev, const float* cam_dev, int32_t B,
                     float* verts_dev, float* joints_dev, float* cam_t_dev, float* kp2d_dev, void* stream) {
    if (int r = check_ready(e, B)) return r;
    if (!rotmat_dev || !betas_dev) return fail(e, THMR_ERR_INVALID, "null buffer");
// ... 48 lines not shown
```

tokenhmr_amd/csrc/ops_abi.hip:

```cpp
#include <hip/hip_runtime.h>

#include <cstring>
#include <map>
#include <mutex>

#include "abi_util.h"
#include "op_gemm_variants.h"
#include "vit_plan.h"

#define THMR_FAIL(code, msg) fail(code, msg)

namespace {

float* op_partial_ws(int dev, void* stream, size_t floats, std::unique_lock<std::mutex>& held) {
    static std::mutex mu;
    static std::map<std::pair<int, void*>, std::pair<float*, size_t>> pool;
    held = std::unique_lock<std::mutex>(mu);
    auto& slot = pool[{dev, stream}];
    if (floats <= slot.second) return slot.first;
    if (slot.first && (hipDeviceSynchronize() != hipSuccess || hipFree(slot.first) != hipSuccess)) return nullptr;
    slot = {nullptr, 0};
    if (hipMalloc(&slot.first, floats * sizeof(float)) != hipSuccess) return slot.first = nullptr;
    slot.second = floats;
    return slot.first;
// ... 110 lines not shown
int thmr_op_layernorm(const float* x, const float* g, const float* b, float* y, int32_t rows, int32_t D, float eps,
                      int32_t relu, void* stream) {
    if (!x || !g || !b || !y) return fail(THMR_ERR_INVALID, "null buffer");
    LAUNCH_OK(launch_layernorm(x, g, b, y, rows, D, eps, relu, static_cast<hipStream_t>(stream)));
    return 0;
}

int thmr_op_vit_attention(const float* qkv, float* out, int32_t B, void* stream) {
    if (!qkv || !out) return fail(THMR_ERR_INVALID, "null buffer");
    LAUNCH_OK(launch_vit_attention(qkv, out, B, static_cast<hipStream_t>(stream)));
    return 0;
}

int thmr_op_vit_attention_split3(const float* qkv, void* out_split, int32_t B, void* stream) {
    if (!qkv || !out_split || B <= 0) return fail(THMR_ERR_INVALID, "bad argument");
    LAUNCH_OK(launch_vit_attention_split3(qkv, out_split, B, static_cast<hipStream_t>(stream)));
    return 0;
}

int thmr_op_vit_attention_b16(const float* qkv, void* out, int32_t B, int32_t out_split, int32_t qt, void* stream) {
    if (!qkv || !out || B <= 0) return fail(THMR_ERR_INVALID, "bad argument");
    LAUNCH_OK(launch_vit_attention_b16(qkv, out, B, out_split != 0, qt, static_cast<hipStream_t>(stream)));
    return 0;
}

int thmr_op_vit_attention_variant(const float* qkv, float* out, int32_t B, int32_t variant, void* stream) {
    if (!qkv || !out) return fail(THMR_ERR_INVALID, "null buffer");
    LAUNCH_OK(launch_vit_attention_variant(qkv, out, B, variant, static_cast<hipStream_t>(stream)));
    return 0;
}

int thmr_op_rot6d(const float* x, float* R, int32_t n, void* stream) {
    if (!x || !R || n < 1) return fail(THMR_ERR_INVALID, "bad argument");
    LAUNCH_OK(launch_rot6d(x, R, n, static_cast<hipStream_t>(stream)));
    return 0;
}

int thmr_op_aa_to_rotmat(const float* aa, float* R, int32_t n, void* stream) {
    if (!aa || !R || n < 1) return fail(THMR_ERR_INVALID, "bad argument");
    LAUNCH_OK(launch_aa_to_rotmat(aa, R, n, static_cast<hipStream_t>(stream)));
    return 0;
}

int thmr_op_splitk_resid_ln(const float* part, int32_t S, int32_t rows, int32_t D, const float* bias, const float* resid, float* xout,
                            const float* gamma, const float* beta, void* y, float eps, int32_t y_is_split3, void* stream) {
    if (!part || !bias || !resid || !xout || !gamma || !beta || !y) return fail(THMR_ERR_INVALID, "splitk_resid_ln: null buffer");
    if (rows <= 0 || S < 1 || D != DIM) return fail(THMR_ERR_INVALID, "splitk_resid_ln: rows >= 1, S >= 1 and D == 1280 are required");
    if (y_is_split3 && S != 2 && S != 4) return fail(THMR_ERR_INVALID, "splitk_resid_ln: the split3 output exists for S = 2 and 4 only");
    LAUNCH_OK(launch_splitk_resid_ln(part, S, rows, D, bias, resid, xout, gamma, beta, static_cast<float*>(y), eps,
                                     static_cast<hipStream_t>(stream), y_is_split3 != 0));
    return 0;
}

int thmr_op_add_ln64(const float* x, const float* y, const float* gamma, const float* beta, float* s_out, float* z_out, int32_t rows,
                     float eps, void* stream) {
    if (!x || !y || !gamma || !beta || !s_out || !z_out) return fail(THMR_ERR_INVALID, "add_ln64: null buffer");
    if (rows <= 0) return fail(THMR_ERR_INVALID, "add_ln64: rows >= 1 is required");
    LAUNCH_OK(launch_add_ln64(x, y, gamma, beta, s_out, z_out, rows, eps, static_cast<hipStream_t>(stream)));
    return 0;
}

int thmr_op_transpose(const float* in, float* out, int32_t Bn, int32_t R, int32_t C, void* stream) {
    if (!in || !out) return fail(THMR_ERR_INVALID, "transpose: null buffer");
    if (Bn <= 0 || R <= 0 || C <= 0 || Bn > 65535 || (R + 31) / 32 > 65535)
        return fail(THMR_ERR_INVALID, "transpose: Bn, R, C >= 1, Bn <= 65535 and R <= 32 * 65535 are required (grid y / z)");
    LAUNCH_OK(launch_transpose(in, out, Bn, R, C, static_cast<hipStream_t>(stream)));
    return 0;
}

int thmr_op_softmax_argmax(const float* logits, float* probs, int32_t* idx, int32_t rows, void* stream) {
    if (!logits) return fail(THMR_ERR_INVALID, "softmax_argmax: null buffer");
    if (!probs && !idx) return fail(THMR_ERR_INVALID, "softmax_argmax: probs and idx are both null");
    if (rows <= 0) return fail(THMR_ERR_INVALID, "softmax_argmax: rows >= 1 is required");
    LAUNCH_OK(launch_softmax_argmax2048(logits, probs, idx, rows, static_cast<hipStream_t>(stream)));
    return 0;
}

int thmr_op_cross_attn(const float* q, const float* kv, int64_t ldkv, int32_t koff, float* out, int32_t B, void* stream) {
    if (!q || !kv || !out) return fail(THMR_ERR_INVALID, "cross_attn: null buffer");
    if (B <= 0 || B > (1 << 24)) return fail(THMR_ERR_INVALID, "cross_attn: 1 <= B <= 2^24 is required");
    if (ldkv <= 0 || koff < 0 || (ldkv % 4) != 0 || (koff % 4) != 0 || (int64_t)koff + 2 * INNER > ldkv)
        return fail(THMR_ERR_INVALID, "cross_attn: ldkv % 4 == 0, koff % 4 == 0 and koff + 1024 <= ldkv are required");
    LAUNCH_OK(launch_cross_attn(q, kv, ldkv, koff, out, B, static_cast<hipStream_t>(stream)));
    return 0;
}

int thmr_op_im2col_patch(const float* img, void* A, int32_t B, int32_t out_split, void* stream) {
    if (!img || !A) return fail(THMR_ERR_INVALID, "im2col_patch: null buffer");
    if (B <= 0) return fail(THMR_ERR_INVALID, "im2col_patch: B >= 1 is required");
    if (out_split) LAUNCH_OK(launch_im2col_patch_split3(img, A, B, static_cast<hipStream_t>(stream)));
    else LAUNCH_OK(launch_im2col_patch(img, static_cast<float*>(A), B, static_cast<hipStream_t>(stream)));
    return 0;
}

int thmr_op_conv3_gather(const float* in, float* out, const int32_t* src, int32_t Bn, int32_t Tin, int32_t Tout, int32_t C, int32_t dil,
                         int32_t prerelu, void* stream) {
    if (!in || !out) return fail(THMR_ERR_INVALID, "conv3_gather: null buffer");
    if (Bn <= 0 || Tin <= 0 || Tout <= 0 || C <= 0 || (C % 4) != 0 || dil < 1)
        return fail(THMR_ERR_INVALID, "conv3_gather: Bn, Tin, Tout >= 1, C % 4 == 0 and dil >= 1 are required");
    if (!src && Tin < Tout) return fail(THMR_ERR_INVALID, "conv3_gather: without an index table Tin >= Tout is required");
    LAUNCH_OK(launch_conv3_gather(in, out, src, Bn, Tin, Tout, C, dil, prerelu, static_cast<hipStream_t>(stream)));
    return 0;
}

int thmr_op_conv_gather(const float* in, float* out, const int32_t* src, int32_t Bn, int32_t Tin, int32_t Tsrc, int32_t Tout, int32_t C,
                        int32_t Cp, int32_t ks, int32_t stride, int32_t pad, void* stream) {
    if (!in || !out) return fail(THMR_ERR_INVALID, "conv_gather: null buffer");
    if (Bn <= 0 || Tin <= 0 || Tsrc <= 0 || Tout <= 0 || C <= 0 || Cp < C || ks < 1 || stride < 1 || pad < 0)
        return fail(THMR_ERR_INVALID, "conv_gather: counts >= 1, Cp >= C, ks >= 1, stride >= 1 and pad >= 0 are required");
    if (!src && Tin < Tsrc) return fail(THMR_ERR_INVALID, "conv_gather: without an index table Tin >= Tsrc is required");
    LAUNCH_OK(launch_conv_gather_general(in, out, src, Bn, Tin, Tsrc, Tout, C, Cp, ks, stride, pad, static_cast<hipStream_t>(stream)));
    return 0;
}

int thmr_op_conv_repack(const float* w, float* wp, int32_t co, int32_t ci, int32_t cp, int32_t kk, void* stream) {
    if (!w || !wp) return fail(THMR_ERR_INVALID, "conv_repack: null buffer");
    if (co <= 0 || ci <= 0 || kk <= 0 || cp < ci) return fail(THMR_ERR_INVALID, "conv_repack: co, ci, kk >= 1 and cp >= ci are required");
    if (cp == ci) LAUNCH_OK(launch_conv_repack(w, wp, co, ci, kk, static_cast<hipStream_t>(stream)));
    else LAUNCH_OK(launch_conv_repack_pad(w, wp, co, ci, cp, kk, static_cast<hipStream_t>(stream)));
    return 0;
}

int thmr_op_vq_argmin_rows(const float* x, const float* dot, const float* cnorm, int32_t* idx, float* dist, int32_t rows, void* stream) {
    if (!x || !dot || !cnorm || !idx) return fail(THMR_ERR_INVALID, "vq_argmin_rows: null buffer");
    if (rows <= 0) return fail(THMR_ERR_INVALID, "vq_argmin_rows: rows >= 1 is required");
    LAUNCH_OK(launch_vq_argmin_rows(x, dot, cnorm, idx, dist, rows, static_cast<hipStream_t>(stream)));
    return 0;
}

int thmr_op_code_norm(const float* cb, float* cn, int32_t ncode, void* stream) {
    if (!cb || !cn) return fail(THMR_ERR_INVALID, "code_norm: null buffer");
    if (ncode <= 0) return fail(THMR_ERR_INVALID, "code_norm: ncode >= 1 is required");
    LAUNCH_OK(launch_code_norm(cb, cn, ncode, static_cast<hipStream_t>(stream)));
    return 0;
}

int thmr_op_vq_stats(const float* x, const float* codebook, const int32_t* idx, int32_t rows, int32_t* code_count, int32_t accumulate,
                     float* partial_scratch, float* commit, float* perplexity, void* stream) {
    if (!x || !codebook || !idx || !code_count || !partial_scratch) return fail(THMR_ERR_INVALID, "vq_stats: null buffer");
    if (rows <= 0) return fail(THMR_ERR_INVALID, "vq_stats: rows >= 1 is required");
    LAUNCH_OK(launch_vq_stats(x, codebook, idx, rows, code_count, accumulate != 0, partial_scratch, commit, perplexity, nullptr,
                              static_cast<hipStream_t>(stream)));
    return 0;
}

int thmr_op_rotmat_to_aa(const float* R, float* aa, int32_t n, void* stream) {
    if (!R || !aa) return fail(THMR_ERR_INVALID, "rotmat_to_aa: null buffer");
    if (n <= 0) return fail(THMR_ERR_INVALID, "rotmat_to_aa: n >= 1 is required");
    LAUNCH_OK(launch_rotmat_to_aa(R, aa, n, static_cast<hipStream_t>(stream)));
    return 0;
}

int thmr_op_head_finish(int32_t kind, const float* ro, int32_t ldro, const float* bpose, const float* init_pose, const float* init_betas,
                        const float* init_cam, float* pose6d, float* rotmat, float* betas, float* cam, float* cam_t, float* focal,
                        float focal_length, float img_size, int32_t B, void* stream) {
    if (kind != 0 && kind != 1) return fail(THMR_ERR_INVALID, "head_finish: kind is 0 (token head) or 1 (HMR2 head)");
    if (!ro || !init_pose || !init_betas || !init_cam || !rotmat || !betas || !cam) return fail(THMR_ERR_INVALID, "head_finish: null buffer");
    if (kind == 0 && !bpose) return fail(THMR_ERR_INVALID, "head_finish: the token head needs the VQ-decoded body pose");
    if (B <= 0) return fail(THMR_ERR_INVALID, "head_finish: B >= 1 is required");
    if (ldro < (kind == 0 ? 31 : THMR_HMR2_RO_ROWS))
        return fail(THMR_ERR_INVALID, "head_finish: ldro is below the read-out's column count (31 token head, 157 HMR2 head)");
    hipStream_t st = static_cast<hipStream_t>(stream);
    if (kind == 0)
        LAUNCH_OK(launch_assemble(ro, ldro, bpose, init_pose, init_betas, init_cam, pose6d, rotmat, betas, cam, cam_t, focal, focal_length,
                                  img_size, B, st));
    else
// ... 243 lines not shown
```

tokenhmr_amd/engine.py:

```python
import ctypes as C

import torch

from . import _cabi
from .config import HMRConfig, RELEASE
from . import weights as W


def _stream_ptr(device):
    return C.c_void_p(torch.cuda.current_stream(device).cuda_stream)


def _ptr(t):
    return C.c_void_p(t.data_ptr()) if t is not None else C.c_void_p(0)


class Engine:

    def __init__(self, cfg: HMRConfig = RELEASE, max_batch: int = 64, device="cuda:0", weight_arena=None, experiments=None,
                 vit_gemm=None, persistent=True):
        self.lib = _cabi.load(exp=experiments)
        self.cfg = cfg
        self._abi = self.lib.thmr_abi_version()
        self.max_batch = int(max_batch)
# ... 196 lines not shown
    def encode_tokens(self, pose6d, want_latent=False):
        pose6d = pose6d.to(self.device, torch.float32).contiguous()
        B = pose6d.shape[0]
        if tuple(pose6d.shape[1:]) != (21, 6):
            raise ValueError(f"pose must be (B,21,6), got {tuple(pose6d.shape)}")
        idx = torch.empty(B, 160, device=self.device, dtype=torch.int32)
        lat = torch.empty(B, 160, 256, device=self.device, dtype=torch.float32) if want_latent else None
        with torch.cuda.device(self.device):
            self._check(self.lib.thmr_encode_tokens(self.h, _ptr(pose6d), B, _ptr(idx), _ptr(lat), _stream_ptr(self.device)), self.h)
        return (idx, lat) if want_latent else idx

    def vq_decode(self, probs):
        probs = probs.to(self.device, torch.float32).contiguous()
        B = probs.shape[0]
        if tuple(probs.shape[1:]) != (160, 2048):
            raise ValueError(f"probs must be (B,160,2048), got {tuple(probs.shape)}")
        pose = torch.empty(B, 21, 6, device=self.device, dtype=torch.float32)
        with torch.cuda.device(self.device):
            self._check(self.lib.thmr_vq_decode(self.h, _ptr(probs), B, _ptr(pose), _stream_ptr(self.device)), self.h)
        return pose

    def vq_decode_idx(self, idx):
        idx = idx.to(self.device, torch.int32).contiguous()
        B = idx.shape[0]
        if idx.dim() != 2 or idx.shape[1] != 160:
            raise ValueError(f"idx must be (B,160), got {tuple(idx.shape)}")
        pose = torch.empty(B, 21, 6, device=self.device, dtype=torch.float32)
        with torch.cuda.device(self.device):
            self._check(self.lib.thmr_vq_decode_idx(self.h, _ptr(idx), B, _ptr(pose), _stream_ptr(self.device)), self.h)
        return pose

    TOKENIZER_OUT = {"idx": ((160,), torch.int32), "latent": ((160, 256), torch.float32), "pose6d": ((21, 6), torch.float32),
                     "rotmat": ((21, 3, 3), torch.float32), "aa": ((21, 3), torch.float32)}

    def tokenizer_roundtrip(self, pose6d, want=("idx", "latent", "pose6d", "rotmat", "commit_loss", "perplexity", "code_count"),
                            outputs=None, accumulate=False):
        pose6d = pose6d.to(self.device, torch.float32).contiguous()
        B = pose6d.shape[0]
        if tuple(pose6d.shape[1:]) != (21, 6):
            raise ValueError(f"pose must be (B,21,6), got {tuple(pose6d.shape)}")
        o = dict(outputs) if outputs is not None else {}
        for k in want:
            if k in o:
                continue
            if k in self.TOKENIZER_OUT:
                shape, dt = self.TOKENIZER_OUT[k]
                o[k] = torch.empty((B,) + shape, device=self.device, dtype=dt)
            elif k in ("commit_loss", "perplexity"):
                o[k] = torch.empty((), device=self.device, dtype=torch.float32)
            elif k == "code_count":
                if accumulate:
                    raise ValueError("accumulate=True needs the caller's code_count in `outputs`")
                o[k] = torch.empty(2048, device=self.device, dtype=torch.int32)
            else:
                raise KeyError(f"unknown round-trip output {k!r}")
        for k, t in o.items():
            shape, dt = self.TOKENIZER_OUT.get(k, ((2048,), torch.int32) if k == "code_count" else ((), torch.float32))
            full = ((B,) + shape) if k in self.TOKENIZER_OUT else shape
            if not (t.is_cuda and t.device == self.device and t.dtype == dt and t.is_contiguous() and tuple(t.shape) == full):
                raise ValueError(f"round-trip output {k!r} must be a contiguous {dt} tensor of shape {full} on {self.device}")
        st = _cabi.TokenizerOut(**{k: o[k].data_ptr() for k in o}, accumulate_counts=1 if accumulate else 0)
        with torch.cuda.device(self.device):
            self._check(self.lib.thmr_tokenizer_roundtrip(self.h, _ptr(pose6d), B, C.byref(st), _stream_ptr(self.device)), self.h)
        return o

    def vq_argmin(self, x, want_dist=False):
        x = x.contiguous()
        rows = x.shape[0]
        idx = torch.empty(rows, device=self.device, dtype=torch.int32)
        dist = torch.empty(rows, 2048, device=self.device, dtype=torch.float32) if want_dist else None
        with torch.cuda.device(self.device):
            self._check(self.lib.thmr_vq_argmin(self.h, _ptr(x), rows, _ptr(idx), _ptr(dist), _stream_ptr(self.device)), self.h)
        return (idx, dist) if want_dist else idx

    VIT_GEMM = {"f32": 0, "split3": 1}

    def set_vit_gemm(self, mode="split3"):
        with torch.cuda.device(self.device):
            self._check(self.lib.thmr_set_vit_gemm(self.h, self.VIT_GEMM[mode], _stream_ptr(self.device)), self.h)

    def vit_gemm(self):
        return {v: k for k, v in self.VIT_GEMM.items()}[self.lib.thmr_get_vit_gemm(self.h)]

    def mode_bytes(self, mode=None):
        m = self.VIT_GEMM[mode] if mode is not None else self.lib.thmr_get_vit_gemm(self.h)
        a, b, c = C.c_size_t(0), C.c_size_t(0), C.c_size_t(0)
        self._check(self.lib.thmr_mode_bytes(C.byref(self._ccfg), m, C.byref(a), C.byref(b), C.byref(c)))
        return {"split_weights": a.value, "split_activations": b.value, "workspace": c.value}

    def prof_enable(self, on=True):
        mode = {"gemm": 2, "fc1": 3}.get(on, 1 if on else 0)
        with torch.cuda.device(self.device):
            self._check(self.lib.thmr_prof_enable(self.h, mode), self.h)

    def prof_collect(self, reset=True):
        arr = (_cabi.ProfEntry * len(_cabi.PROF_NAMES))()
        with torch.cuda.device(self.device):
            self._check(self.lib.thmr_prof_collect(self.h, arr, 1 if reset else 0), self.h)
        return {n: dict(ms=arr[i].ms, flops=arr[i].flops, bytes=arr[i].bytes, launches=arr[i].launches)
                for i, n in enumerate(_cabi.PROF_NAMES)}
```

tokenhmr_amd/ops.py:

```python
import ctypes as C

import torch

from . import _cabi

EPI = {"none": 0, "bias": 1, "bias_gelu": 2, "bias_relu": 3, "bias_resid": 4, "bias_qscale": 5, "bias_pos": 6}
VARIANT = {"auto": -1, "128x128reg": 0, "128x160reg": 1, "skinny": 2, "128x128": 7, "128x160": 8, "64x64": 9, "128x96": 10, "tiny": 11, "64x128": 12, "128x64": 13, "ring16": 120}
VARIANT.update({f"ring{r}" + (f"/k{1 << j}" if j else ""): 100 + (10 if r == 8 else 0) + j for r in (4, 8) for j in range(5)})
VARIANT.update({f"{t}/k{k}": 100 * k + c for t, c in (("auto", 0), ("128x128", 7), ("128x160", 8), ("128x96", 10), ("64x128", 12), ("128x64", 13)) for k in (2, 4)})


_EXP = None


class experiments_build:

    def __enter__(self):
        global _EXP
        self._old, _EXP = _EXP, True
        return self

    def __exit__(self, *a):
        global _EXP
        _EXP = self._old
# ... 153 lines not shown

def rot6d_to_rotmat(x):
    _req(x)
    x2 = x.reshape(-1, 6).contiguous()
    n = x2.shape[0]
    R = torch.empty(n, 3, 3, device=x.device, dtype=torch.float32)
    with torch.cuda.device(x.device):
        _check(_L().thmr_op_rot6d(_p(x2), _p(R), n, _s(x)))
    return R


def aa_to_rotmat(theta):
    _req(theta)
    x = theta.reshape(-1, 3).contiguous()
    n = x.shape[0]
    R = torch.empty(n, 3, 3, device=theta.device, dtype=torch.float32)
    with torch.cuda.device(theta.device):
        _check(_L().thmr_op_aa_to_rotmat(_p(x), _p(R), n, _s(theta)))
    return R


def _req_i32(*ts):
    for t in ts:
        if t is not None and not (t.is_cuda and t.dtype == torch.int32 and t.is_contiguous()):
            raise ValueError("index tables are contiguous int32 CUDA tensors")


def splitk_resid_ln(part, bias, resid, gamma, beta, eps, y_split3=False, inplace=False):
    _req(part, bias, resid, gamma, beta)
    S, rows, D = part.shape
    if resid.shape != (rows, D):
        raise ValueError("resid is (rows, D)")
    xout = resid if inplace else torch.empty(rows, D, device=part.device, dtype=torch.float32)
    y = (torch.empty(rows, D // 8, 3, 8, device=part.device, dtype=torch.int16) if y_split3
         else torch.empty(rows, D, device=part.device, dtype=torch.float32))
    with torch.cuda.device(part.device):
        _check(_L().thmr_op_splitk_resid_ln(_p(part), S, rows, D, _p(bias), _p(resid), _p(xout), _p(gamma), _p(beta), _p(y), float(eps),
                                            int(y_split3), _s(part)))
    return xout, y


def add_ln64(x, y, gamma, beta, eps):
    _req(x, y, gamma, beta)
    if x.shape != y.shape or x.shape[-1] != 64:
        raise ValueError("add_ln64 needs two (rows, 64) tensors")
    s, z = torch.empty_like(x), torch.empty_like(x)
    with torch.cuda.device(x.device):
        _check(_L().thmr_op_add_ln64(_p(x), _p(y), _p(gamma), _p(beta), _p(s), _p(z), x.numel() // 64, float(eps), _s(x)))
    return s, z


def transpose(x, out=None):
    _req(x, out)
    Bn, R, Cc = x.shape
    if out is None:
        out = torch.empty(Bn, Cc, R, device=x.device, dtype=torch.float32)
    elif out.shape != (Bn, Cc, R):
        raise ValueError("out must be (Bn, C, R)")
    with torch.cuda.device(x.device):
        _check(_L().thmr_op_transpose(_p(x), _p(out), Bn, R, Cc, _s(x)))
    return out


def softmax_argmax(logits, probs=True, idx=True):
    _req(logits)
    rows = logits.shape[0]
    if logits.shape != (rows, 2048):
        raise ValueError("softmax_argmax needs (rows, 2048) logits")
    p = torch.empty_like(logits) if probs else None
    i = torch.empty(rows, device=logits.device, dtype=torch.int32) if idx else None
    with torch.cuda.device(logits.device):
        _check(_L().thmr_op_softmax_argmax(_p(logits), _p(p), _p(i), rows, _s(logits)))
    return p, i


def cross_attn(q, kv, koff=0):
    _req(q, kv)
    B = q.shape[0]
    if q.shape != (B, 512) or kv.dim() != 2 or kv.shape[0] != B * 192:
        raise ValueError("cross_attn needs q (B, 512) and kv (B * 192, ldkv)")
    out = torch.empty(B, 512, device=q.device, dtype=torch.float32)
    with torch.cuda.device(q.device):
        _check(_L().thmr_op_cross_attn(_p(q), _p(kv), kv.shape[1], int(koff), _p(out), B, _s(q)))
    return out


def im2col_patch(img, out_split=False):
    _req(img)
    B = img.shape[0]
    if img.shape != (B, 3, 256, 256):
        raise ValueError("im2col_patch needs (B, 3, 256, 256)")
    out = (torch.empty(B * 192, 96, 3, 8, device=img.device, dtype=torch.int16) if out_split
           else torch.empty(B * 192, 768, device=img.device, dtype=torch.float32))
    with torch.cuda.device(img.device):
        _check(_L().thmr_op_im2col_patch(_p(img), _p(out), B, int(out_split), _s(img)))
    return out


def conv3_gather(x, Tout, src=None, dil=1, prerelu=False, out=None):
    _req(x, out)
    _req_i32(src)
    Bn, Tin, Cc = x.shape
    if src is not None and src.numel() != Tout:
        raise ValueError("src holds one index per output position")
    if out is None:
        out = torch.empty(Bn, Tout, 3 * Cc, device=x.device, dtype=torch.float32)
    elif out.shape != (Bn, Tout, 3 * Cc):
        raise ValueError("out must be (Bn, Tout, 3 C)")
    with torch.cuda.device(x.device):
        _check(_L().thmr_op_conv3_gather(_p(x), _p(out), _p(src), Bn, Tin, int(Tout), Cc, int(dil), int(prerelu), _s(x)))
    return out


def conv_gather(x, Tout, ks, stride, pad, Cp=None, src=None, Tsrc=None, out=None):
    _req(x, out)
    _req_i32(src)
    Bn, Tin, Cc = x.shape
    Cp = Cc if Cp is None else int(Cp)
    Tsrc = (Tin if src is None else src.numel()) if Tsrc is None else int(Tsrc)
    if src is not None and src.numel() != Tsrc:
        raise ValueError("src holds one index per resampled position")
    if out is None:
        out = torch.empty(Bn, Tout, ks * Cp, device=x.device, dtype=torch.float32)
    elif out.shape != (Bn, Tout, ks * Cp):
        raise ValueError("out must be (Bn, Tout, ks Cp)")
    with torch.cuda.device(x.device):
        _check(_L().thmr_op_conv_gather(_p(x), _p(out), _p(src), Bn, Tin, Tsrc, int(Tout), Cc, Cp, int(ks), int(stride), int(pad), _s(x)))
    return out


def conv_repack(w, cp=None):
    _req(w)
    co, ci, kk = w.shape
    cp = ci if cp is None else int(cp)
    out = torch.empty(co, kk * cp, device=w.device, dtype=torch.float32)
    with torch.cuda.device(w.device):
        _check(_L().thmr_op_conv_repack(_p(w), _p(out), co, ci, cp, kk, _s(w)))
    return out


def vq_argmin_rows(x, dot, cnorm, want_dist=True):
    _req(x, dot, cnorm)
    rows = x.shape[0]
    if x.shape != (rows, 256) or dot.shape != (rows, 2048) or cnorm.shape != (2048,):
        raise ValueError("vq_argmin_rows needs x (rows, 256), dot (rows, 2048), cnorm (2048)")
    idx = torch.empty(rows, device=x.device, dtype=torch.int32)
    dist = torch.empty(rows, 2048, device=x.device, dtype=torch.float32) if want_dist else None
    with torch.cuda.device(x.device):
        _check(_L().thmr_op_vq_argmin_rows(_p(x), _p(dot), _p(cnorm), _p(idx), _p(dist), rows, _s(x)))
    return idx, dist


def code_norm(cb):
    _req(cb)
    n = cb.shape[0]
    if cb.shape != (n, 256):
        raise ValueError("code_norm needs (ncode, 256)")
    cn = torch.empty(n, device=cb.device, dtype=torch.float32)
    with torch.cuda.device(cb.device):
        _check(_L().thmr_op_code_norm(_p(cb), _p(cn), n, _s(cb)))
    return cn


def head_finish(kind, ro, init_pose, init_betas, init_cam, bpose=None, focal_length=5000.0, img_size=256.0,
                want_pose6d=True, want_cam_t=True, want_focal=True):
    _req(ro, init_pose, init_betas, init_cam, bpose)
# ... 118 lines not shown
```

Baseline: 875.4 crops/s.

## Fold cross-attention K/V projections into decoder via query-side weight folding

Instead of projecting the whole ViT context (B*192 tokens x 1280) into K and V for all six decoder layers with a split3 GEMM, the decoder now folds Wk into the single query (u = q·Wk), scores the raw context directly, forms a softmax-weighted context sum per chunk, and only then applies Wv. This removes the large dec_kv GEMM and its split3 conversion, which is significant work with one query token per sample. The cost is extra per-layer stages inside the fused decoder, which must reread the context each layer, plus workspace and fp32-MFMA numerics that differ from the split3 path.

```diff
diff --git a/include/tokenhmr_hip.h b/include/tokenhmr_hip.h
--- a/include/tokenhmr_hip.h
+++ b/include/tokenhmr_hip.h
@@ -140,6 +140,8 @@
 } thmr_vit_plan_desc;
 int thmr_debug_vit_plan(const thmr_config* cfg, int32_t vit_gemm_mode, int32_t B, int32_t streams_available, thmr_vit_plan_desc* out);
 
+int thmr_debug_kv_fold(thmr_engine* e, int32_t B);
+
 int thmr_vit_forward(thmr_engine* e, const float* img_dev, int32_t B, float* feats_dev , void* stream);
 int thmr_head_forward(thmr_engine* e, const float* ctx_dev , int32_t B, const thmr_outputs* out, void* stream);
 int thmr_lbs_forward(thmr_engine* e, const float* rotmat_dev , const float* betas_dev ,
@@ -191,6 +193,8 @@
 int thmr_op_transpose(const float* in_dev, float* out_dev, int32_t Bn, int32_t R, int32_t C, void* stream);
 int thmr_op_softmax_argmax(const float* logits_dev, float* probs_or_null, int32_t* idx_or_null, int32_t rows, void* stream);
 int thmr_op_cross_attn(const float* q_dev, const float* kv_dev, int64_t ldkv, int32_t koff, float* out_dev, int32_t B, void* stream);
+#define THMR_CROSS_ATTN_FOLD_WS_FLOATS 51264
+int thmr_op_cross_attn_fold(const float* q_dev, const float* ctx_dev, const float* wkv_dev, float* out_dev, void* ws_dev, int32_t B, void* stream);
 int thmr_op_im2col_patch(const float* img_dev, void* A_dev, int32_t B, int32_t out_split, void* stream);
 int thmr_op_conv3_gather(const float* in_dev, float* out_dev, const int32_t* src_or_null, int32_t Bn, int32_t Tin, int32_t Tout,
                          int32_t C, int32_t dil, int32_t prerelu, void* stream);
diff --git a/tokenhmr_amd/_cabi.py b/tokenhmr_amd/_cabi.py
--- a/tokenhmr_amd/_cabi.py
+++ b/tokenhmr_amd/_cabi.py
@@ -162,6 +162,8 @@
 ROWOPS_SYMBOLS = ("thmr_op_splitk_resid_ln", "thmr_op_add_ln64", "thmr_op_transpose", "thmr_op_softmax_argmax", "thmr_op_cross_attn",
                   "thmr_op_im2col_patch", "thmr_op_conv3_gather", "thmr_op_conv_gather", "thmr_op_conv_repack", "thmr_op_vq_argmin_rows",
                   "thmr_op_code_norm", "thmr_op_head_finish", "thmr_op_decoder_init")
+
+KV_FOLD_SYMBOLS = ("thmr_op_cross_attn_fold", "thmr_debug_kv_fold")
 
 TOKENIZER_RT_SYMBOLS = ("thmr_vq_decode_idx", "thmr_tokenizer_roundtrip", "thmr_op_vq_stats", "thmr_op_rotmat_to_aa")
 
@@ -204,7 +206,7 @@
             getattr(lib, name).restype = restypes[ret]
     older = isinstance(exp, str) and lib.thmr_abi_version() in (3, 4)
     missing = [s for s in sorted(declared) if not hasattr(lib, s) and not (older and s in ("thmr_mode_bytes",))
-               and not (isinstance(exp, str) and s in ("thmr_renderer_sheet", "thmr_debug_vit_plan") + ROWOPS_SYMBOLS + TOKENIZER_RT_SYMBOLS + FRAMES_SYMBOLS + JPEG_SYMBOLS)]
+               and not (isinstance(exp, str) and s in ("thmr_renderer_sheet", "thmr_debug_vit_plan") + ROWOPS_SYMBOLS + KV_FOLD_SYMBOLS + TOKENIZER_RT_SYMBOLS + FRAMES_SYMBOLS + JPEG_SYMBOLS)]
     if missing:
         raise RuntimeError(f"libtokenhmr_hip.so lacks symbols declared in tokenhmr_hip.h: {missing}")
     vp, i32, i64, f32, sz = C.c_void_p, C.c_int32, C.c_int64, C.c_float, C.c_size_t
@@ -255,6 +257,9 @@
         lib.thmr_op_code_norm.argtypes = [vp, vp, i32, vp]
         lib.thmr_op_head_finish.argtypes = [i32, vp, i32, vp, vp, vp, vp, vp, vp, vp, vp, vp, vp, f32, f32, i32, vp]
         lib.thmr_op_decoder_init.argtypes = [vp, vp, vp, i32, i32, vp]
+    if hasattr(lib, "thmr_op_cross_attn_fold"):
+        lib.thmr_op_cross_attn_fold.argtypes = [vp, vp, vp, vp, vp, i32, vp]
+        lib.thmr_debug_kv_fold.argtypes = [vp, i32]
     if hasattr(lib, "thmr_tokenizer_roundtrip"):
         lib.thmr_vq_decode_idx.argtypes = [vp, vp, i32, vp, vp]
         lib.thmr_tokenizer_roundtrip.argtypes = [vp, vp, i32, C.POINTER(TokenizerOut), vp]
diff --git a/tokenhmr_amd/csrc/common.h b/tokenhmr_amd/csrc/common.h
--- a/tokenhmr_amd/csrc/common.h
+++ b/tokenhmr_amd/csrc/common.h
@@ -255,12 +255,16 @@
 struct DecLayerW {
     const float *n0w, *n0b, *wv, *wo1, *bo1;
     const float *n1w, *n1b, *wq, *wo2, *bo2;
+    const float *wkc, *wvc;
     const float *n2w, *n2b, *w1, *b1, *w2, *b2;
 };
 struct DecParams {
     DecLayerW L[6];
     const float *tok_bias, *pos;
     const float* kv;
+    const float* ctx;
+    float *fu, *fz, *fml;
+    int kv_fold;
     const float *ro_w, *ro_b, *mt_w, *mt_b;
     float *dx, *dv, *dq, *dca, *dff, *ro, *mt;
     unsigned* sync;
@@ -280,6 +284,8 @@
 constexpr int THMR_HMR2_RO_ROWS = 157, THMR_HMR2_RO_LD = 160;
 int launch_decoder_fused(const DecParams& p, hipStream_t s, int head = THMR_HEAD_TOKEN);
 int decoder_max_coresident_blocks(int device, int head = THMR_HEAD_TOKEN);
+size_t cross_attn_fold_ws_floats(int B);
+int launch_cross_attn_fold(const float* q, const float* ctx, const float* wkv, float* out, float* ws, int B, hipStream_t s);
 int launch_hmr2_finish(const float* ro, int ldro, const float* init_pose, const float* init_betas, const float* init_cam, float* pose6d,
                        float* rotmat, float* betas, float* cam, float* cam_t, float* focal, float focal_length, float img_size, int B,
                        hipStream_t s);
diff --git a/tokenhmr_amd/csrc/decoder_fused.hip b/tokenhmr_amd/csrc/decoder_fused.hip
--- a/tokenhmr_amd/csrc/decoder_fused.hip
+++ b/tokenhmr_amd/csrc/decoder_fused.hip
@@ -270,7 +270,13 @@
 
 namespace {
 
-__device__ __forceinline__ void cross_attn_stage(const DecParams& p, int layer, int tid, float* pl ) {
+__device__ __forceinline__ int stage_local(int tid) {
+    asm volatile("" : "+v"(tid));
+    return tid;
+}
+
+__device__ __forceinline__ void cross_attn_stage(const DecParams& p, int layer, int tid_, float* pl ) {
+    const int tid = stage_local(tid_);
     const int lane = tid & 63, l15 = lane & 15, g = lane >> 4;
     const int gwave = __builtin_amdgcn_readfirstlane(tid >> 6) * gridDim.x + blockIdx.x;
     for (int item = gwave; item < p.B * NHEAD; item += gridDim.x * NWAVE) {
@@ -358,6 +364,216 @@
     }
 }
 
+constexpr int CTXD = 1280, FOLD_CHUNKS = 4, FOLD_TOK = TOKK / FOLD_CHUNKS;
+constexpr int FOLD_LDS = NWAVE * FOLD_TOK * NHEAD + NHEAD * FOLD_TOK;
+constexpr int FOLD_VS = CTXD / NWAVE / 16;
+static_assert(FOLD_TOK == 48 && CTXD % (NWAVE * 32) == 0, "stage A's lane mapping");
+
+__device__ __forceinline__ void st_dev2(float* p, float a, float b) {
+    union { unsigned long long u; f32x2 f; } v;
+    v.f = f32x2{a, b};
+    __hip_atomic_store(reinterpret_cast<unsigned long long*>(p), v.u, __ATOMIC_RELAXED, __HIP_MEMORY_SCOPE_AGENT);
+}
+
+__device__ __forceinline__ void fold_u_load_w(f32x4 (&w)[8], const float* __restrict__ Wk, int item, int tid) {
+    const int lane = tid & 63, wave = __builtin_amdgcn_readfirstlane(tid >> 6), l15 = lane & 15, g = lane >> 4;
+    const int hn = item % 40, h = hn / 5, nb = hn % 5;
+    const float* wp = Wk + (int64_t)(h * 64 + g * 4) * CTXD + nb * 256 + wave * 32 + l15;
+#pragma unroll
+    for (int j = 0; j < 2; ++j)
+#pragma unroll
+        for (int s = 0; s < 4; ++s)
+#pragma unroll
+            for (int t = 0; t < 4; ++t) w[j * 4 + s][t] = wp[(s * 16 + t) * CTXD + j * 16];
+}
+__device__ __forceinline__ void fold_u_stage(const float* q, const float* __restrict__ Wk, float* u, int B, int tid_) {
+    const int tid = stage_local(tid_);
+    const int lane = tid & 63, wave = __builtin_amdgcn_readfirstlane(tid >> 6), l15 = lane & 15, g = lane >> 4;
+    const int nsub = (B + 15) >> 4;
+    for (int item = blockIdx.x; item < 40 * nsub; item += gridDim.x) {
+        const int hn = item % 40, h = hn / 5, nb = hn % 5, m0 = (item / 40) * 16;
+        f32x4 w[8];
+        fold_u_load_w(w, Wk, item, tid);
+        const float* ap = q + (int64_t)min(m0 + l15, B - 1) * INNER + h * 64 + g * 4;
+        f32x4 a[4];
+#pragma unroll
+        for (int s = 0; s < 4; ++s) a[s] = ld_dev4(ap + s * 16);
+#pragma unroll
+        for (int j = 0; j < 2; ++j) {
+            f32x4 acc = {0.f, 0.f, 0.f, 0.f};
+#pragma unroll
+            for (int s = 0; s < 4; ++s)
+#pragma unroll
+                for (int t = 0; t < 4; ++t) acc = __builtin_amdgcn_mfma_f32_16x16x4f32(a[s][t], w[j * 4 + s][t], acc, 0, 0, 0);
+            const int n = nb * 256 + wave * 32 + j * 16 + l15;
+#pragma unroll
+            for (int r = 0; r < 4; ++r) {
+                const int m = m0 + g * 4 + r;
+                if (m < B) st_dev(u + ((int64_t)m * NHEAD + h) * CTXD + n, acc[r]);
+            }
+        }
+    }
+}
+
+__device__ __forceinline__ void fold_a_stage(const float* __restrict__ ctx, const float* u, float* zp, float* ml, int B, int tid_, float* lds) {
+    const int tid = stage_local(tid_);
+    const int lane = tid & 63, wave = __builtin_amdgcn_readfirstlane(tid >> 6), l15 = lane & 15, g = lane >> 4;
+    float* sp = lds;
+    float* ps = lds + NWAVE * FOLD_TOK * NHEAD;
+    for (int item = blockIdx.x; item < B * FOLD_CHUNKS; item += gridDim.x) {
+        const int b = item >> 2, c = item & 3;
+        const float* cb = ctx + ((int64_t)b * TOKK + c * FOLD_TOK) * CTXD;
+        {
+            const int kbeg = wave * (CTXD / NWAVE);
+            const float* up = u + ((int64_t)b * NHEAD + (l15 & 7)) * CTXD + kbeg + g * 4;
+            f32x4 uq[FOLD_VS];
+#pragma unroll
+            for (int s = 0; s < FOLD_VS; ++s) uq[s] = ld_dev4(up + s * 16);
+#pragma unroll
+            for (int tt = 0; tt < 3; ++tt) {
+                const float* xp = cb + (int64_t)(tt * 16 + l15) * CTXD + kbeg + g * 4;
+                f32x4 xq[FOLD_VS];
+#pragma unroll
+                for (int s = 0; s < FOLD_VS; ++s) xq[s] = *reinterpret_cast<const f32x4*>(xp + s * 16);
+                f32x4 acc = {0.f, 0.f, 0.f, 0.f};
+#pragma unroll
+                for (int s = 0; s < FOLD_VS; ++s)
+#pragma unroll
+                    for (int t = 0; t < 4; ++t) acc = __builtin_amdgcn_mfma_f32_16x16x4f32(xq[s][t], uq[s][t], acc, 0, 0, 0);
+                if (l15 < NHEAD) {
+#pragma unroll
+                    for (int r = 0; r < 4; ++r) sp[(wave * FOLD_TOK + tt * 16 + g * 4 + r) * NHEAD + l15] = acc[r];
+                }
+            }
+        }
+        __syncthreads();
+        if (tid < FOLD_TOK * NHEAD) {
+            float s = sp[tid];
+#pragma unroll
+            for (int w = 1; w < NWAVE; ++w) s += sp[w * FOLD_TOK * NHEAD + tid];
+            ps[(tid & 7) * FOLD_TOK + (tid >> 3)] = s * 0.125f;
+        }
+        __syncthreads();
+        {
+            const float sv = lane < FOLD_TOK ? ps[wave * FOLD_TOK + lane] : -INFINITY;
+            const float m = wave_max(sv);
+            const float e = lane < FOLD_TOK ? expf(sv - m) : 0.f;
+            const float l = wave_sum(e);
+            if (lane < FOLD_TOK) ps[wave * FOLD_TOK + lane] = e;
+            if (lane == 0) st_dev2(ml + ((int64_t)item * NHEAD + wave) * 2, m, l);
+        }
+        __syncthreads();
+        {
+            float pa[FOLD_TOK / 4];
+#pragma unroll
+            for (int ks = 0; ks < FOLD_TOK / 4; ++ks) pa[ks] = l15 < NHEAD ? ps[l15 * FOLD_TOK + ks * 4 + g] : 0.f;
+            const float* xp = cb + (int64_t)g * CTXD + wave * (CTXD / NWAVE) + l15 * 2;
+            f32x4 acc[5][2];
+#pragma unroll
+            for (int pt = 0; pt < 5; ++pt) acc[pt][0] = acc[pt][1] = f32x4{0.f, 0.f, 0.f, 0.f};
+#pragma unroll
+            for (int half = 0; half < 2; ++half) {
+                f32x2 x[6][5];
+#pragma unroll
+                for (int k = 0; k < 6; ++k)
+#pragma unroll
+                    for (int pt = 0; pt < 5; ++pt) x[k][pt] = *reinterpret_cast<const f32x2*>(xp + (int64_t)((half * 6 + k) * 4) * CTXD + pt * 32);
+#pragma unroll
+                for (int k = 0; k < 6; ++k)
+#pragma unroll
+                    for (int pt = 0; pt < 5; ++pt) {
+                        acc[pt][0] = __builtin_amdgcn_mfma_f32_16x16x4f32(pa[half * 6 + k], x[k][pt][0], acc[pt][0], 0, 0, 0);
+                        acc[pt][1] = __builtin_amdgcn_mfma_f32_16x16x4f32(pa[half * 6 + k], x[k][pt][1], acc[pt][1], 0, 0, 0);
+                    }
+            }
+            if (g < 2) {
+                float* zo = zp + ((int64_t)item * NHEAD + g * 4) * CTXD + wave * (CTXD / NWAVE) + l15 * 2;
+#pragma unroll
+                for (int r = 0; r < 4; ++r)
+#pragma unroll
+                    for (int pt = 0; pt < 5; ++pt) st_dev2(zo + r * CTXD + pt * 32, acc[pt][0][r], acc[pt][1][r]);
+            }
+        }
+        __syncthreads();
+    }
+}
+
+__device__ __forceinline__ void fold_v_stage(const float* zp, const float* ml, const float* __restrict__ Wv, float* out, int B, int tid_,
+                                             float (*red)[64][4]) {
+    const int tid = stage_local(tid_);
+    const int lane = tid & 63, wave = __builtin_amdgcn_readfirstlane(tid >> 6), l15 = lane & 15, g = lane >> 4;
+    const int kbeg = wave * (CTXD / NWAVE);
+    const int ngrp = (B + 7) >> 3;
+    constexpr int HS = FOLD_VS / 2;
+    for (int item = blockIdx.x; item < 32 * ngrp; item += gridDim.x) {
+        const int ct = item & 31, h = ct >> 2, n0 = ct * 16, m0 = (item >> 5) * 8;
+        const int m = m0 + l15;
+        const bool row = l15 < 8 && m < B;
+        const float* wp = Wv + (int64_t)(n0 + l15) * CTXD + kbeg + g * 4;
+        const float* zb = zp + ((int64_t)(row ? m : 0) * FOLD_CHUNKS * NHEAD + h) * CTXD + kbeg + g * 4;
+        float wc[FOLD_CHUNKS] = {0.f, 0.f, 0.f, 0.f}, inv = 0.f;
+        if (row) {
+            const float* mp = ml + ((int64_t)m * FOLD_CHUNKS * NHEAD + h) * 2;
+            float mc[FOLD_CHUNKS], lc[FOLD_CHUNKS];
+#pragma unroll
+            for (int c = 0; c < FOLD_CHUNKS; ++c) {
+                union { unsigned long long u; f32x2 f; } v;
+                v.u = __hip_atomic_load(reinterpret_cast<const unsigned long long*>(mp + c * NHEAD * 2), __ATOMIC_RELAXED, __HIP_MEMORY_SCOPE_AGENT);
+                mc[c] = v.f.x; lc[c] = v.f.y;
+            }
+            const float mx = fmaxf(fmaxf(mc[0], mc[1]), fmaxf(mc[2], mc[3]));
+            float lsum = 0.f;
+#pragma unroll
+            for (int c = 0; c < FOLD_CHUNKS; ++c) {
+                wc[c] = expf(mc[c] - mx);
+                lsum = c == 0 ? wc[0] * lc[0] : fmaf(wc[c], lc[c], lsum);
+            }
+            inv = 1.0f / lsum;
+        }
+        f32x4 acc = {0.f, 0.f, 0.f, 0.f};
+#pragma unroll 1
+        for (int sh = 0; sh < 2; ++sh) {
+            f32x4 wq[HS], xq[HS];
+#pragma unroll
+            for (int s = 0; s < HS; ++s) wq[s] = *reinterpret_cast<const f32x4*>(wp + (sh * HS + s) * 16);
+            if (row) {
+#pragma unroll
+                for (int c = 0; c < FOLD_CHUNKS; ++c)
+#pragma unroll
+                    for (int s = 0; s < HS; ++s) {
+                        const f32x4 z = ld_dev4(zb + (int64_t)c * NHEAD * CTXD + (sh * HS + s) * 16);
+#pragma unroll
+                        for (int t = 0; t < 4; ++t) xq[s][t] = c == 0 ? wc[0] * z[t] : fmaf(wc[c], z[t], xq[s][t]);
+                    }
+#pragma unroll
+                for (int s = 0; s < HS; ++s)
+#pragma unroll
+                    for (int t = 0; t < 4; ++t) xq[s][t] *= inv;
+            } else {
+#pragma unroll
+                for (int s = 0; s < HS; ++s) xq[s] = f32x4{0.f, 0.f, 0.f, 0.f};
+            }
+#pragma unroll
+            for (int s = 0; s < HS; ++s)
+#pragma unroll
+                for (int t = 0; t < 4; ++t) acc = __builtin_amdgcn_mfma_f32_16x16x4f32(xq[s][t], wq[s][t], acc, 0, 0, 0);
+        }
+        *reinterpret_cast<f32x4*>(&red[wave][lane][0]) = acc;
+        __syncthreads();
+        if (wave == 0 && g < 2) {
+            f32x4 v = *reinterpret_cast<const f32x4*>(&red[0][lane][0]);
+#pragma unroll
+            for (int w = 1; w < NWAVE; ++w) v += *reinterpret_cast<const f32x4*>(&red[w][lane][0]);
+#pragma unroll
+            for (int r = 0; r < 4; ++r) {
+                const int mo = m0 + g * 4 + r;
+                if (mo < B) st_dev(out + (int64_t)mo * INNER + n0 + l15, v[r]);
+            }
+        }
+        __syncthreads();
+    }
+}
+
 __device__ __forceinline__ bool mixer_cluster_stage(const DecParams& p, GridSync& gs, int tid, volatile int* s_ok, float* Y, float* U, float* Xl,
                                                     float* redbuf) {
     using namespace mixer;
@@ -416,6 +632,9 @@
     __shared__ __attribute__((aligned(16))) float mixY[TOKEN ? mixer::T * mixer::LD : 4];
     __shared__ __attribute__((aligned(16))) float mixU[TOKEN ? mixer::H * mixer::LD : 4];
     __shared__ __attribute__((aligned(16))) float mixX[TOKEN ? 80 * mixer::LD : 4];
+    __shared__ __attribute__((aligned(16))) float foldown[TOKEN ? 4 : FOLD_LDS];
+    float* foldlds = TOKEN ? mixY : foldown;
+    static_assert(!TOKEN || mixer::T * mixer::LD >= FOLD_LDS, "stage A's LDS fits the mixer's row buffer");
     __shared__ float mixred[mixer::NW];
     static_assert(mixer::NW == NWAVE, "the distributed mixer tail uses the decoder kernel's 8 waves");
     __shared__ __attribute__((aligned(16))) float red[NWAVE][64][4];
@@ -436,7 +655,7 @@
     const int B = p.B;
     unsigned long long* stamp = (p.timeline && blockIdx.x == 0 && tid == 0) ? reinterpret_cast<unsigned long long*>(p.sync + 16) : nullptr;
     int nstamp = 0;
-#define THMR_STAMP() do { if (stamp) stamp[nstamp++] = wall_clock64(); } while (0)
+#define THMR_STAMP() do { if (stamp && nstamp < 120) stamp[nstamp++] = wall_clock64(); } while (0)
     THMR_STAMP();
 
     for (int i = blockIdx.x * (NWAVE * 64) + tid; i < B * E; i += gridDim.x * NWAVE * 64) {
@@ -461,10 +680,25 @@
         gemv_stage<true, 0>(p.dx, E, w.n1w, w.n1b, w.wq, E, nullptr, nullptr, p.dq, INNER, INNER, B, red, &rowstat, tid, pre);
         THMR_STAMP();
         pre.item = -1;
-        if (!(ok = grid_barrier(gs, tid, &s_ok))) break;
-        THMR_STAMP();
-        cross_attn_stage(p, l, tid, &red[__builtin_amdgcn_readfirstlane(tid >> 6)][0][0]);
-        THMR_STAMP();
+        if (p.kv_fold) {
+            if (!(ok = grid_barrier(gs, tid, &s_ok))) break;
+            THMR_STAMP();
+            fold_u_stage(p.dq, w.wkc, p.fu, B, tid);
+            THMR_STAMP();
+            if (!(ok = grid_barrier(gs, tid, &s_ok))) break;
+            THMR_STAMP();
+            fold_a_stage(p.ctx, p.fu, p.fz, p.fml, B, tid, foldlds);
+            THMR_STAMP();
+            if (!(ok = grid_barrier(gs, tid, &s_ok))) break;
+            THMR_STAMP();
+            fold_v_stage(p.fz, p.fml, w.wvc, p.dca, B, tid, red);
+            THMR_STAMP();
+        } else {
+            if (!(ok = grid_barrier(gs, tid, &s_ok))) break;
+            THMR_STAMP();
+            cross_attn_stage(p, l, tid, &red[__builtin_amdgcn_readfirstlane(tid >> 6)][0][0]);
+            THMR_STAMP();
+        }
         if (!(ok = grid_barrier(gs, tid, &s_ok, [&] { prefetch_w(pre, w.wo2, INNER, E, B, tid); }))) break;
         THMR_STAMP();
         gemv_stage<false, 4>(p.dca, INNER, nullptr, nullptr, w.wo2, INNER, w.bo2, p.dx, p.dx, E, E, B, red, &rowstat, tid, pre);
@@ -509,6 +743,34 @@
     }
 }
 
+}
+
+namespace {
+__global__ __launch_bounds__(NWAVE * 64) void fold_u_kernel(const float* q, const float* Wk, float* u, int B) {
+    fold_u_stage(q, Wk, u, B, threadIdx.x);
+}
+__global__ __launch_bounds__(NWAVE * 64) void fold_a_kernel(const float* ctx, const float* u, float* zp, float* ml, int B) {
+    __shared__ __attribute__((aligned(16))) float lds[FOLD_LDS];
+    fold_a_stage(ctx, u, zp, ml, B, threadIdx.x, lds);
+}
+__global__ __launch_bounds__(NWAVE * 64) void fold_v_kernel(const float* zp, const float* ml, const float* Wv, float* out, int B) {
+    __shared__ __attribute__((aligned(16))) float red[NWAVE][64][4];
+    fold_v_stage(zp, ml, Wv, out, B, threadIdx.x, red);
+}
+}
+
+size_t cross_attn_fold_ws_floats(int B) { return (size_t)B * (NHEAD * CTXD + FOLD_CHUNKS * NHEAD * CTXD + FOLD_CHUNKS * NHEAD * 2); }
+
+int launch_cross_attn_fold(const float* q, const float* ctx, const float* wkv, float* out, float* ws, int B, hipStream_t s) {
+    if (B < 1) return -1;
+    float* u = ws;
+    float* zp = u + (size_t)B * NHEAD * CTXD;
+    float* ml = zp + (size_t)B * FOLD_CHUNKS * NHEAD * CTXD;
+    auto grid = [](int64_t items) { return dim3((unsigned)(items < 1024 ? items : 1024)); };
+    hipLaunchKernelGGL(fold_u_kernel, grid(40 * (int64_t)((B + 15) / 16)), dim3(NWAVE * 64), 0, s, q, wkv, u, B);
+    hipLaunchKernelGGL(fold_a_kernel, grid((int64_t)B * FOLD_CHUNKS), dim3(NWAVE * 64), 0, s, ctx, u, zp, ml, B);
+    hipLaunchKernelGGL(fold_v_kernel, grid(32 * (int64_t)((B + 7) / 8)), dim3(NWAVE * 64), 0, s, zp, ml, wkv + (size_t)INNER * CTXD, out, B);
+    return hipGetLastError() == hipSuccess ? 0 : -2;
 }
 
 constexpr int kDecMinGrid = 128;
diff --git a/tokenhmr_amd/csrc/engine.hip b/tokenhmr_amd/csrc/engine.hip
--- a/tokenhmr_amd/csrc/engine.hip
+++ b/tokenhmr_amd/csrc/engine.hip
@@ -679,14 +679,18 @@
     return vq_decode_convs(e, B, bpose, st);
 }
 
+static bool kv_fold_of(bool fused_head, const VitPlan& plan) { return fused_head && plan.to_kv.kind != THMR_GEMM_F32_TILE; }
+
 int head_forward(thmr_engine* e, const float* ctx, int B, const thmr_outputs* out, hipStream_t st) {
     auto& so = e->so;
     const int M = B * TOK;
     float* big = e->S(so.big);
     const int ldkv = e->dec_depth * 2 * INNER;
-    {
+    const bool fused_head = !e->legacy_head && B <= kFusedHeadMaxB;
+    const VitPlan plan = plan_of(e, B);
+    const bool kv_fold = kv_fold_of(fused_head, plan);
+    if (!kv_fold) {
         ProfScope ps(e, st, THMR_PROF_DEC_KV, 2.0 * M * DIM * (double)ldkv, 4.0 * ((double)M * DIM + (double)ldkv * DIM + (double)M * ldkv));
-        const VitPlan plan = plan_of(e, B);
         if (plan.to_kv.kind != THMR_GEMM_F32_TILE) {
             LAUNCH_OK(launch_split3(ctx, DIM, e->split_act, DIM, M, DIM, st));
             GemmArgs a = mk(reinterpret_cast<const float*>(e->split_act), DIM, reinterpret_cast<const float*>(e->kv_s), DIM, nullptr, nullptr, 0, big, ldkv, M, ldkv, DIM);
@@ -703,11 +707,15 @@
     const std::string C = "smpl_head.decpose.";
     float* ro = e->S(so.ro);
     float *mt = e->S(so.mt), *cf = e->S(so.cf), *cf2 = e->S(so.cf2);
-    const bool fused_head = !e->legacy_head && B <= kFusedHeadMaxB;
     bool mixer_in_decoder = false;
     if (fused_head) {
         DecParams d = e->dec;
         d.B = B;
+        if (kv_fold) {
+            d.kv_fold = 1;
+            d.ctx = ctx;
+            d.fu = big; d.fz = d.fu + (size_t)B * 8 * DIM; d.fml = d.fz + (size_t)B * 4 * 8 * DIM;
+        }
         if (e->hmr2) {
             d.mixer_cluster = 0;
             LAUNCH_OK(launch_decoder_fused(d, st, THMR_HEAD_HMR2));
@@ -1313,12 +1321,14 @@
             w.n1w = e->W(p + "1.norm.weight"); w.n1b = e->W(p + "1.norm.bias");
             w.wq = e->W(p + "1.fn.to_q.weight");
             w.wo2 = e->W(p + "1.fn.to_out.0.weight"); w.bo2 = e->W(p + "1.fn.to_out.0.bias");
+            w.wkc = e->warena + e->o_kv_all + (size_t)l * 2 * INNER * DIM; w.wvc = w.wkc + (size_t)INNER * DIM;
             w.n2w = e->W(p + "2.norm.weight"); w.n2b = e->W(p + "2.norm.bias");
             w.w1 = e->W(p + "2.fn.net.0.weight"); w.b1 = e->W(p + "2.fn.net.0.bias");
             w.w2 = e->W(p + "2.fn.net.3.weight"); w.b2 = e->W(p + "2.fn.net.3.bias");
         }
         d.tok_bias = e->W(T + "to_token_embedding.bias"); d.pos = e->W(T + "pos_embedding");
         d.kv = e->S(e->so.big); d.ldkv = (int64_t)e->dec_depth * 2 * INNER;
+        d.kv_fold = 0; d.ctx = nullptr; d.fu = d.fz = d.fml = nullptr;
         d.ro_w = e->warena + e->o_ro_w; d.ro_b = e->warena + e->o_ro_b;
         if (!e->hmr2) { d.mt_w = e->W("smpl_head.decpose.mixer_trans.ff.0.weight"); d.mt_b = e->W("smpl_head.decpose.mixer_trans.ff.0.bias"); }
         d.dx = e->S(e->so.dx); d.dv = e->S(e->so.dv); d.dq = e->S(e->so.dq); d.dca = e->S(e->so.dca); d.dff = e->S(e->so.dff);
@@ -1548,6 +1558,13 @@
     return 0;
 }
 
+int thmr_debug_kv_fold(thmr_engine* e, int32_t B) {
+    if (!e) return fail(e, THMR_ERR_INVALID, "null engine");
+    if (!e->finalized) return fail(e, THMR_ERR_STATE, "weights not finalized");
+    if (B < 1 || B > e->max_batch) return fail(e, THMR_ERR_INVALID, "batch outside [1, max_batch]");
+    return kv_fold_of(!e->legacy_head && B <= kFusedHeadMaxB, plan_of(e, B)) ? 1 : 0;
+}
+
 int thmr_debug_vit_plan(const thmr_config* cfg, int32_t vit_gemm_mode, int32_t B, int32_t streams_available, thmr_vit_plan_desc* out) {
     if (int r = validate_cfg(cfg)) return r;
     if (vit_gemm_mode != 0 && vit_gemm_mode != 1) return fail(nullptr, THMR_ERR_INVALID, "vit gemm mode must be 0 or 1");
diff --git a/tokenhmr_amd/csrc/ops_abi.hip b/tokenhmr_amd/csrc/ops_abi.hip
--- a/tokenhmr_amd/csrc/ops_abi.hip
+++ b/tokenhmr_amd/csrc/ops_abi.hip
@@ -216,6 +216,16 @@
     if (ldkv <= 0 || koff < 0 || (ldkv % 4) != 0 || (koff % 4) != 0 || (int64_t)koff + 2 * INNER > ldkv)
         return fail(THMR_ERR_INVALID, "cross_attn: ldkv % 4 == 0, koff % 4 == 0 and koff + 1024 <= ldkv are required");
     LAUNCH_OK(launch_cross_attn(q, kv, ldkv, koff, out, B, static_cast<hipStream_t>(stream)));
+    return 0;
+}
+
+int thmr_op_cross_attn_fold(const float* q, const float* ctx, const float* wkv, float* out, void* ws, int32_t B, void* stream) {
+    if (!q || !ctx || !wkv || !out || !ws) return fail(THMR_ERR_INVALID, "cross_attn_fold: null buffer");
+    if (B <= 0 || B > (1 << 16)) return fail(THMR_ERR_INVALID, "cross_attn_fold: 1 <= B <= 2^16 is required");
+    if ((reinterpret_cast<uintptr_t>(q) | reinterpret_cast<uintptr_t>(ctx) | reinterpret_cast<uintptr_t>(wkv) | reinterpret_cast<uintptr_t>(ws)) & 15)
+        return fail(THMR_ERR_INVALID, "cross_attn_fold: q, ctx, wkv and ws must be 16-byte aligned");
+    if (cross_attn_fold_ws_floats(B) != (size_t)B * THMR_CROSS_ATTN_FOLD_WS_FLOATS) return fail(THMR_ERR_INVALID, "cross_attn_fold: internal: workspace size");
+    LAUNCH_OK(launch_cross_attn_fold(q, ctx, wkv, out, static_cast<float*>(ws), B, static_cast<hipStream_t>(stream)));
     return 0;
 }
 
diff --git a/tokenhmr_amd/engine.py b/tokenhmr_amd/engine.py
--- a/tokenhmr_amd/engine.py
+++ b/tokenhmr_amd/engine.py
@@ -302,6 +302,12 @@
     def vit_gemm(self):
         return {v: k for k, v in self.VIT_GEMM.items()}[self.lib.thmr_get_vit_gemm(self.h)]
 
+    def kv_fold(self, B):
+        r = self.lib.thmr_debug_kv_fold(self.h, int(B))
+        if r < 0:
+            self._check(r, self.h)
+        return r == 1
+
     def mode_bytes(self, mode=None):
         m = self.VIT_GEMM[mode] if mode is not None else self.lib.thmr_get_vit_gemm(self.h)
         a, b, c = C.c_size_t(0), C.c_size_t(0), C.c_size_t(0)
diff --git a/tokenhmr_amd/ops.py b/tokenhmr_amd/ops.py
--- a/tokenhmr_amd/ops.py
+++ b/tokenhmr_amd/ops.py
@@ -259,6 +259,18 @@
     out = torch.empty(B, 512, device=q.device, dtype=torch.float32)
     with torch.cuda.device(q.device):
         _check(_L().thmr_op_cross_attn(_p(q), _p(kv), kv.shape[1], int(koff), _p(out), B, _s(q)))
+    return out
+
+
+def cross_attn_fold(q, ctx, wkv):
+    _req(q, ctx, wkv)
+    B = q.shape[0]
+    if q.shape != (B, 512) or ctx.shape != (B, 192, 1280) or wkv.shape != (1024, 1280):
+        raise ValueError("cross_attn_fold needs q (B, 512), ctx (B, 192, 1280) and wkv (1024, 1280)")
+    out = torch.empty(B, 512, device=q.device, dtype=torch.float32)
+    ws = torch.empty(B * 51264, device=q.device, dtype=torch.float32)
+    with torch.cuda.device(q.device):
+        _check(_L().thmr_op_cross_attn_fold(_p(q), _p(ctx), _p(wkv), _p(out), _p(ws), B, _s(q)))
     return out
 
 
```

Measured after the change: 880.8 crops/s (median of 6 runs). Within noise of the previous version (+0.6%).
